# peternara/FashionVisualExpl-recommend

Measured on AMD Instinct MI355X. Metric: BPR triplets/sec, higher is better.
Workload: dtype bf16

## Files before the change

fashionvisualexpl_recommend_amd/_ffi.py:

```python
import ctypes as C
import os

HERE = os.path.dirname(os.path.abspath(__file__))
LIB_PATH = os.environ.get("BPRX_LIB") or os.path.join(HERE, "libbprx.so")
ABI_VERSION = 6
FLAG_EXPORT_USER_GRAD = 1
FLAG_EXPORT_ITEM_GRAD = 2
FLAG_DENSE_ALLREDUCE = 4
FLAG_ADAM_SWEEP, FLAG_ADAM_LAZY = 8, 16

MODEL = {"bprmf": 0, "vbpr": 1}
OPTIMIZER = {"sgd": 0, "adam_tf23": 1}
FEAT_DTYPE = {"fp32": 0, "bf16": 1, "fp8": 2}
E_INVALID, E_STATE = -1, -2
E_RANGE = -4
PHASES = ["cast_Et", "proj_fwd", "triplet_grad", "proj_bwd", "reduce_parts", "apply", "dense_update", "loss_reduce", "item_seg", "seg_alloc", "row_count", "adam_catchup"]


class BprxError(RuntimeError):
    def __init__(self, code, msg):
        super().__init__("libbprx error %d: %s" % (code, msg))
        self.code = code


class Config(C.Structure):
    _fields_ = [("abi_version", C.c_int32), ("model", C.c_int32), ("num_users", C.c_int32), ("num_items", C.c_int32),
                ("embed_k", C.c_int32), ("embed_d", C.c_int32), ("feat_dim", C.c_int32), ("feat_dtype", C.c_int32),
                ("optimizer", C.c_int32), ("device", C.c_int32), ("max_batch", C.c_int64),
                ("lr", C.c_float), ("reg", C.c_float), ("beta1", C.c_float), ("beta2", C.c_float),
                ("epsilon", C.c_float), ("flags", C.c_int32), ("feat_scale", C.c_float)]


FACTORED_FIELDS = ["Ea", "Eb", "A", "Ap", "m_Ea", "v_Ea", "m_Eb", "v_Eb", "m_A", "v_A", "m_Ap", "v_Ap"]


class Factored(C.Structure):
    _fields_ = [("feat_dim_a", C.c_int32), ("feat_dim_b", C.c_int32), ("embed_a", C.c_int32), ("embed_b", C.c_int32),
                ("neg_bias_reg", C.c_float)] + [(n, C.c_void_p) for n in FACTORED_FIELDS]


ACF_WEIGHTS = ["component.W_0_u", "component.W_0_i", "component.b_0", "component.W_1", "component.b_1",
               "item.W_0_u", "item.W_0_iv", "item.W_0_ip", "item.W_0_ix", "item.b_0", "item.W_1", "item.b_1"]


ACF_GRADIENT = {"detached": 0, "full": 1}


class Acf(C.Structure):
    _fields_ = [("feat_m", C.c_int32), ("feat_c", C.c_int32), ("width_c", C.c_int32), ("width_i", C.c_int32),
                ("feat_dtype", C.c_int32), ("F", C.c_void_p), ("train_ptr", C.c_void_p), ("train_items", C.c_void_p),
                ("eval_ptr", C.c_void_p), ("eval_items", C.c_void_p), ("Pi", C.c_void_p), ("m_Pi", C.c_void_p),
                ("v_Pi", C.c_void_p), ("w", C.c_void_p * 12), ("m_w", C.c_void_p * 12), ("v_w", C.c_void_p * 12)]


AF_WEIGHTS = ["color.W1", "color.b1", "color.W2", "edges.conv", "edges.conv_b", "edges.W2", "class.W1", "class.b1", "class.W2",
              "attention.W_1", "attention.b_1", "attention.W_2", "attention.b_2"]


class Attentive(C.Structure):
    _fields_ = [("dim_color", C.c_int32), ("dim_class", C.c_int32), ("width", C.c_int32), ("dropout", C.c_float),
                ("seed", C.c_uint64), ("edges", C.c_void_p), ("color", C.c_void_p), ("cls", C.c_void_p),
                ("w", C.c_void_p * 13), ("m_w", C.c_void_p * 13), ("v_w", C.c_void_p * 13)]


TABLE_FIELDS = ["Gu", "Gi", "Bi", "Tu", "F", "E", "Bp", "m_Gu", "v_Gu", "m_Gi", "v_Gi", "m_Bi", "v_Bi",
                "m_Tu", "v_Tu", "m_E", "v_E", "m_Bp", "v_Bp"]


class Tables(C.Structure):
    _fields_ = [(n, C.c_void_p) for n in TABLE_FIELDS]


_lib = None


def lib():
    global _lib
    if _lib is not None:
        return _lib
    import torch
    if not os.path.exists(LIB_PATH):
        raise ImportError("libbprx.so not found at %s: build it with `python -m fashionvisualexpl_recommend_amd.build` "
                          "(hipcc --offload-arch=gfx950); there is no CPU fallback" % LIB_PATH)
    L = C.CDLL(LIB_PATH)
    vp, i32, i64, u32, f32 = C.c_void_p, C.c_int32, C.c_int64, C.c_uint32, C.c_float
    sig = {
        "bprx_abi_version": (C.c_int, []),
        "bprx_create": (C.c_int, [C.POINTER(Config), C.POINTER(vp)]),
        "bprx_destroy": (C.c_int, [vp]),
        "bprx_last_error": (C.c_char_p, [vp]),
        "bprx_bind_tables": (C.c_int, [vp, C.POINTER(Tables)]),
        "bprx_bind_factored": (C.c_int, [vp, C.POINTER(Tables), C.POINTER(Factored)]),
        "bprx_explain_pairs": (C.c_int, [vp, vp, vp, i64, vp, vp]),
        "bprx_bind_acf": (C.c_int, [vp, C.POINTER(Tables), C.POINTER(Acf)]),
        "bprx_acf_profiles": (C.c_int, [vp, vp, i64, vp, vp, vp, vp]),
        "bprx_acf_explain": (C.c_int, [vp, vp, vp, i64, vp, vp, i32, vp, vp, vp, vp, vp, vp, vp, vp, vp, vp]),
        "bprx_acf_set_gradient": (C.c_int, [vp, C.c_int]),
        "bprx_acf_get_gradient": (C.c_int, [vp]),
        "bprx_bind_attentive": (C.c_int, [vp, C.POINTER(Tables), C.POINTER(Attentive)]),
        "bprx_af_encode": (C.c_int, [vp, vp, i64, vp, vp]),
        "bprx_af_attention_pairs": (C.c_int, [vp, vp, vp, i64, vp, vp, vp]),
        "bprx_af_explain": (C.c_int, [vp, vp, vp, i64, i32, vp, vp, vp, vp, vp, vp, vp]),
        "bprx_af_score_block": (C.c_int, [vp, C.c_int32, C.c_int32, vp, vp, vp]),
        "bprx_af_dropout_mask": (C.c_int, [vp, i64, i64, vp, vp]),
        "bprx_af_get_step": (i64, [vp]),
        "bprx_af_set_step": (C.c_int, [vp, i64]),
        "bprx_set_hyper": (C.c_int, [vp, f32, f32]),
        "bprx_tables_dirty": (C.c_int, [vp, vp]),
        "bprx_set_adam_step": (C.c_int, [vp, i64, vp]),
        "bprx_get_adam_step": (i64, [vp]),
        "bprx_adam_is_lazy": (C.c_int, [vp]),
        "bprx_sync_adam": (C.c_int, [vp, vp]),
        "bprx_score_pairs": (C.c_int, [vp, vp, vp, i64, vp, vp]),
        "bprx_step": (C.c_int, [vp, vp, vp, vp, i64, vp, vp]),
        "bprx_step_begin": (C.c_int, [vp, vp, vp, vp, i64, vp]),
        "bprx_step_begin_sparse": (C.c_int, [vp, vp, vp, vp, i64, vp]),
        "bprx_step_begin_dense": (C.c_int, [vp, vp]),
        "bprx_dense_grad": (C.c_int, [vp, C.POINTER(vp), C.POINTER(i64)]),
        "bprx_step_end": (C.c_int, [vp, vp, vp]),
        "bprx_step_project": (C.c_int, [vp, vp]),
        "bprx_user_grad": (C.c_int, [vp, C.POINTER(vp), C.POINTER(vp)]),
        "bprx_clear_user_grad": (C.c_int, [vp, i64, i32, vp]),
        "bprx_item_grad": (C.c_int, [vp, C.POINTER(vp), C.POINTER(vp)]),
        "bprx_clear_item_grad": (C.c_int, [vp, i64, i32, vp]),
        "bprx_scatter_add": (C.c_int, [vp, i32, i32, vp, vp, i64, f32, vp]),
        "bprx_route_reset": (C.c_int, [vp, i64, vp, i32, vp]),
        "bprx_route_plan": (C.c_int, [vp, i64, vp, i64, i32, i32, i32, i32, vp, vp, vp, vp, vp, vp]),
        "bprx_route_gather": (C.c_int, [vp, i32, vp, i32, i32, vp, i64, vp, vp, vp]),
        "bprx_route_unpack": (C.c_int, [vp, vp, i64, vp, i32, vp, i32, vp, vp, i32, vp]),
        "bprx_route_gather_checked": (C.c_int, [vp, i32, vp, i32, i32, vp, i64, vp, vp, vp, vp]),
        "bprx_route_unpack_checked": (C.c_int, [vp, vp, i64, vp, i32, vp, i32, vp, vp, i32, vp, vp]),
        "bprx_route_pack": (C.c_int, [vp, i32, vp, i32, vp, i64, vp, vp, vp, i32, f32, vp, vp, i64, vp, i32, vp]),
        "bprx_route_scatter_add": (C.c_int, [vp, i32, vp, i32, i32, vp, vp, i64, f32, vp, vp]),
        "bprx_score_block": (C.c_int, [vp, i32, i32, vp, vp]),
        "bprx_eval_users": (C.c_int, [vp, i32, i32, vp, vp, vp, vp, vp, i32, vp, vp]),
        "bprx_topk": (C.c_int, [vp, i32, i32, vp, vp, vp, i32, vp, vp, vp, vp]),
        "bprx_eval_pos": (C.c_int, [vp, i32, i32, vp, i32, i32, vp, vp, vp, vp]),
        "bprx_eval_counts": (C.c_int, [vp, i32, i32, vp, i32, i32, vp, vp, vp, vp, vp, vp, vp]),
        "bprx_eval_finish": (C.c_int, [vp, i32, i32, i32, vp, vp, vp, i32, vp, vp]),
        "bprx_sync_check": (C.c_int, [vp, vp]),
        "bprx_probe_stream_read": (i64, [vp, i64, vp, vp]),
        "bprx_probe_stream_read_nt": (i64, [vp, i64, vp, vp]),
        "bprx_probe_row_gather": (i64, [vp, i64, i32, vp, i64, i32, vp, vp]),
        "bprx_profile_enable": (C.c_int, [vp, C.c_int]),
        "bprx_profile_read": (C.c_int, [vp, vp, vp]),
        "bprx_sample_philox": (C.c_int, [vp, vp, vp, i64, i32, C.c_uint64, C.c_uint64, i64, vp, vp, vp, vp]),
        "bprx_user_msg_floats": (C.c_int64, [vp, i64]),
        "bprx_pack_user_msg": (C.c_int, [vp, vp, i64, i64, vp, vp]),
        "bprx_apply_user_msgs": (C.c_int, [vp, vp, i32, i64, C.c_float, vp]),
        "bprx_sum_dense_parts": (C.c_int, [vp, vp, i32, vp]),
        "bprx_epoch_prepare": (C.c_int, [C.c_uint64, u32, i32, vp, vp, vp, vp]),
        "bprx_epoch_slots": (C.c_int, [vp, i32, vp, i64, vp]),
        "bprx_sample_epoch": (C.c_int, [vp, vp, vp, vp, vp, i32, i32, C.c_uint64, u32, i64, i64, vp, vp, vp, vp]),
        "bprx_index_pass_kind": (C.c_int, [vp]),
        "bprx_adam_rows": (C.c_int, [vp, vp, vp, vp, i64, C.c_float, C.c_float, C.c_float, C.c_float, vp]),
        "bprx_step_lr": (C.c_int, [vp, vp]),
        "bprx_sample_philox_h": (C.c_int, [vp, vp, vp, vp, i64, i32, C.c_uint64, C.c_uint64, i64, vp, vp, vp, i64, i64, vp]),
        "bprx_sample_epoch_h": (C.c_int, [vp, vp, vp, vp, vp, vp, i32, i32, C.c_uint64, u32, i64, i64, vp, vp, vp, i64, i64, vp]),
        "bprx_sampler_create": (C.c_int, [vp, vp, i32, i32, C.POINTER(vp)]),
        "bprx_sampler_destroy": (C.c_int, [vp]),
        "bprx_sampler_count": (i64, [vp, i32, i32]),
        "bprx_sampler_ref_stream": (i64, [vp, i32, i32, u32, u32, vp, vp, vp, i64]),
    }
    for name, (res, args) in sig.items():
        fn = getattr(L, name)
        fn.restype, fn.argtypes = res, args
    if L.bprx_abi_version() != ABI_VERSION:
        raise ImportError("libbprx.so ABI %d != binding ABI %d" % (L.bprx_abi_version(), ABI_VERSION))
    _lib = L
    return L


EXPORTS = ["bprx_abi_version", "bprx_create", "bprx_destroy", "bprx_last_error", "bprx_bind_tables", "bprx_bind_factored", "bprx_explain_pairs", "bprx_bind_acf", "bprx_acf_profiles", "bprx_acf_explain", "bprx_acf_set_gradient", "bprx_acf_get_gradient", "bprx_bind_attentive", "bprx_af_encode", "bprx_af_attention_pairs", "bprx_af_explain",
           "bprx_af_score_block", "bprx_af_dropout_mask", "bprx_af_get_step", "bprx_af_set_step", "bprx_set_hyper", "bprx_tables_dirty",
           "bprx_set_adam_step", "bprx_get_adam_step", "bprx_adam_is_lazy", "bprx_sync_adam", "bprx_score_pairs", "bprx_step", "bprx_step_begin",
           "bprx_step_begin_sparse", "bprx_step_begin_dense", "bprx_sum_dense_parts",
           "bprx_dense_grad", "bprx_step_end", "bprx_step_project", "bprx_user_grad", "bprx_clear_user_grad", "bprx_item_grad", "bprx_clear_item_grad",
           "bprx_scatter_add", "bprx_route_reset", "bprx_route_plan", "bprx_route_gather", "bprx_route_unpack", "bprx_route_gather_checked",
           "bprx_route_unpack_checked", "bprx_route_pack",
           "bprx_route_scatter_add", "bprx_score_block", "bprx_eval_users", "bprx_eval_pos", "bprx_eval_counts", "bprx_eval_finish", "bprx_topk", "bprx_sync_check", "bprx_probe_stream_read", "bprx_probe_stream_read_nt", "bprx_probe_row_gather", "bprx_profile_enable",
           "bprx_profile_read", "bprx_sample_philox", "bprx_epoch_prepare", "bprx_epoch_slots", "bprx_sample_epoch", "bprx_sample_philox_h", "bprx_sample_epoch_h", "bprx_index_pass_kind", "bprx_adam_rows", "bprx_step_lr", "bprx_user_msg_floats", "bprx_pack_user_msg",
           "bprx_apply_user_msgs", "bprx_sampler_create",
           "bprx_sampler_destroy", "bprx_sampler_count", "bprx_sampler_ref_stream"]


def check(handle, rc):
    if rc < 0:
        msg = lib().bprx_last_error(handle)
        raise BprxError(rc, msg.decode() if msg else "?")
    return rc
```

fashionvisualexpl_recommend_amd/csrc/bprx_api.hip:

```cpp
#include <math.h>
#include <stdlib.h>
#include <algorithm>
#include <new>

#include "bprx_internal.h"
#include <utility>

static char g_create_err[512] = "";

static int check_ready(bprx_handle *h, int64_t B);

extern "C" int bprx_abi_version(void) { return BPRX_ABI_VERSION; }

extern "C" const char *bprx_last_error(const bprx_handle *h) { return h ? h->err : g_create_err; }

template <typename T>
static hipError_t dalloc_zero(T **p, size_t n) {
  *p = nullptr;
  if (n == 0) return hipSuccess;
  hipError_t e = hipMalloc((void **)p, n * sizeof(T));
  if (e != hipSuccess) return e;
  return hipMemset(*p, 0, n * sizeof(T));
}

static int env_int(const char *name, int fallback) {
  const char *e = getenv(name);
  return e ? atoi(e) : fallback;
}

static void free_scratch(bprx_handle *h) {
  void *ptrs[] = {h->dGu, h->dGi, h->dBi, h->dTu, h->flagU, h->flagI, h->lossb, h->loss_acc, h->errflag,
                  h->P,   h->W,   h->Wb, h->Ppair, h->Et, h->EtF, h->EtS, h->dEp, h->part, h->qs, h->Ft, h->seg_rank, h->seg_cnt, h->seg_ptr, h->seg_cursor, h->seg_lead, h->seg_ent, h->hot_done, h->uslot_of, h->ulist, h->uold, h->own8, h->loc8, h->cntU, h->cntI, h->ilist, h->ilist_n, h->lastU, h->lastI, h->lr_hist, h->slist, h->slist_n, h->msg_cursor, h->msg_next, h->gF};
  for (void *p : ptrs)
    if (p) (void)hipFree(p);
}

extern "C" int bprx_create(const bprx_config *cfg, bprx_handle **out) {
#define CFAIL(code, ...)                                        \
  do {                                                          \
    snprintf(g_create_err, sizeof(g_create_err), __VA_ARGS__);  \
    return (code);                                              \
  } while (0)
  if (!cfg || !out) CFAIL(BPRX_E_INVALID, "bprx_create: null argument");
  *out = nullptr;
  if (cfg->abi_version != BPRX_ABI_VERSION)
    CFAIL(BPRX_E_INVALID, "bprx_create: abi_version %d, library is %d", cfg->abi_version, BPRX_ABI_VERSION);
  if (cfg->model != BPRX_MODEL_BPRMF && cfg->model != BPRX_MODEL_VBPR) CFAIL(BPRX_E_INVALID, "unknown model %d", cfg->model);
  if (cfg->optimizer != BPRX_OPT_SGD && cfg->optimizer != BPRX_OPT_ADAM_TF23)
    CFAIL(BPRX_E_INVALID, "unknown optimizer %d", cfg->optimizer);
  if (cfg->num_users <= 0 || cfg->num_items <= 0 || cfg->embed_k <= 0 || cfg->max_batch <= 0)
    CFAIL(BPRX_E_INVALID, "num_users, num_items, embed_k and max_batch must be positive");
  const bool vb = cfg->model == BPRX_MODEL_VBPR;
  if (vb) {
    if (cfg->embed_d <= 0 || cfg->feat_dim <= 0) CFAIL(BPRX_E_INVALID, "VBPR needs embed_d > 0 and feat_dim > 0");
    if (cfg->embed_d > 271) CFAIL(BPRX_E_INVALID, "embed_d %d > 271 unsupported", cfg->embed_d);
    if (cfg->feat_dtype != BPRX_F_FP32 && cfg->feat_dtype != BPRX_F_BF16 && cfg->feat_dtype != BPRX_F_FP8)
      CFAIL(BPRX_E_INVALID, "unknown feat_dtype");
    if (cfg->feat_dtype == BPRX_F_BF16 && cfg->feat_dim % 128 != 0)
      CFAIL(BPRX_E_INVALID, "bf16 features need feat_dim %% 128 == 0 (got %d)", cfg->feat_dim);
    if (cfg->feat_dtype == BPRX_F_FP8 && cfg->feat_dim % 256 != 0)
      CFAIL(BPRX_E_INVALID, "fp8 features need feat_dim %% 256 == 0 (got %d)", cfg->feat_dim);
    if (cfg->feat_dtype == BPRX_F_FP8 && !(cfg->feat_scale > 0.f)) CFAIL(BPRX_E_INVALID, "fp8 features need feat_scale > 0");
  }
  const bool exported = cfg->flags & (BPRX_FLAG_EXPORT_USER_GRAD | BPRX_FLAG_EXPORT_ITEM_GRAD);
  bool adam_lazy = false;
  if (cfg->optimizer == BPRX_OPT_ADAM_TF23) {
    const double chain_us = 20.0 * (double)cfg->num_users / (double)cfg->max_batch * 0.45;
    const double sweep_us =
        ((double)cfg->num_users * (cfg->embed_k + (vb ? cfg->embed_d : 0)) + (double)cfg->num_items * (cfg->embed_k + 1)) * 24.0 / 4e6;
    adam_lazy = exported ? true : chain_us < sweep_us;
    if (cfg->flags & BPRX_FLAG_ADAM_SWEEP) adam_lazy = false;
    if (cfg->flags & BPRX_FLAG_ADAM_LAZY) adam_lazy = true;
    adam_lazy = env_int("BPRX_ADAM_LAZY", adam_lazy) != 0;
  }
  if (exported && cfg->optimizer != BPRX_OPT_SGD && !adam_lazy)
    CFAIL(BPRX_E_INVALID, "BPRX_FLAG_EXPORT_*_GRAD with adam_tf23 needs the lazy form (BPRX_ADAM_LAZY != 0)");
  if ((cfg->flags & BPRX_FLAG_EXPORT_ITEM_GRAD) && cfg->model != BPRX_MODEL_BPRMF)
    CFAIL(BPRX_E_INVALID, "BPRX_FLAG_EXPORT_ITEM_GRAD is for BPRMF (VBPR keeps its items and features local)");
  hipError_t e = hipSetDevice(cfg->device);
  if (e != hipSuccess) CFAIL(BPRX_E_HIP, "hipSetDevice(%d): %s", cfg->device, hipGetErrorString(e));

  bprx_handle *h = new (std::nothrow) bprx_handle();
  if (!h) CFAIL(BPRX_E_NOMEM, "out of host memory");
  memset(h, 0, sizeof(*h));
#define HFAIL(code, ...)         \
  do {                           \
    bprx_destroy(h);             \
    CFAIL(code, __VA_ARGS__);    \
  } while (0)
  h->cfg = *cfg;
  h->adam_lazy = adam_lazy;
  h->neg_bias_reg = 0.1f;
  if (!vb) { h->cfg.embed_d = 0; h->cfg.feat_dim = 0; }
  const size_t U = cfg->num_users, I = cfg->num_items, k = cfg->embed_k, d = h->cfg.embed_d, D = h->cfg.feat_dim;
  const size_t MB = cfg->max_batch;
  bool ok = true;
#define A(call) ok = ok && ((e = (call)) == hipSuccess)
  A(dalloc_zero(&h->dGu, U * k));
  A(dalloc_zero(&h->dGi, I * k));
  A(dalloc_zero(&h->dBi, I));
  A(dalloc_zero(&h->flagU, U));
  A(dalloc_zero(&h->flagI, I));
  A(dalloc_zero(&h->lossb, MB));
  A(dalloc_zero(&h->loss_acc, (size_t)BPRX_DENSE_BLOCKS));
  A(dalloc_zero(&h->errflag, (size_t)1));
  if (cfg->flags & BPRX_FLAG_EXPORT_USER_GRAD) A(dalloc_zero(&h->msg_cursor, (size_t)2));
  A(dalloc_zero(&h->cntU, U));
  A(dalloc_zero(&h->cntI, I));
  if (vb) {
    h->PS = 16 * (int)((d + 1 + 15) / 16);
    const size_t PS = h->PS;
    {
      hipDeviceProp_t prop;
      const int ncu = hipGetDeviceProperties(&prop, cfg->device) == hipSuccess ? prop.multiProcessorCount : 256;
      const int mr = (int)((D + 255) / 256);
      h->SK = (ncu + mr - 1) / mr;
      if (cfg->feat_dtype == BPRX_F_FP8 && PS / 16 <= 9) h->SK *= 2;
    }
    if (h->SK > 64) h->SK = 64;
    if (h->SK < 1) h->SK = 1;
    h->fwd_variant = env_int("BPRX_FWD_VARIANT", 4);
    A(dalloc_zero(&h->dTu, U * d));
    A(dalloc_zero(&h->P, I * PS));
    A(dalloc_zero(&h->W, I * PS));
    A(dalloc_zero((uint16_t **)&h->Wb, I * PS));
    A(dalloc_zero(&h->Ppair, MB * PS));
    A(dalloc_zero((uint16_t **)&h->Et, PS * D));
    A(dalloc_zero((uint16_t **)&h->EtF, PS * D));
    if (cfg->feat_dtype == BPRX_F_FP8 && PS / 16 >= 10) A(dalloc_zero((uint8_t **)&h->EtS, PS * D));
    A(dalloc_zero(&h->dEp, D * d + D));
    A(dalloc_zero(&h->part, (size_t)h->SK * D * PS));
    A(dalloc_zero(&h->qs, (size_t)4));
    if (cfg->feat_dtype != BPRX_F_FP32)
      A(dalloc_zero((uint8_t **)&h->Ft, (size_t)((I + 31) / 32 * 32) * D * (cfg->feat_dtype == BPRX_F_FP8 ? 1 : 2)));
  }
#undef A
  if (!ok) HFAIL(BPRX_E_NOMEM, "scratch allocation failed: %s", hipGetErrorString(e));
  {
    const bool fits = k % 4 == 0 && d % 4 == 0 && k <= 256 && d <= 256;
    h->seg_policy = (fits && !(cfg->flags & BPRX_FLAG_EXPORT_ITEM_GRAD)) ? std::min(std::max(env_int("BPRX_ITEM_MODE", 1), 0), 2) : 0;
    h->item_mode = 0;
    if (h->seg_policy) {
      h->seg_lead_cap = (int64_t)(I + 8192 + 4 * 1024 + 2 * MB / 64 + 64 + 64);
      h->seg_ent_cap = (int64_t)(6 * MB + 64 * 1024 + 2048);
      h->idx8_shift = 0;
      for (int sh = 8; sh <= 13 && !h->idx8_shift; ++sh)
        if ((((int64_t)I - 1) >> sh) <= 255) h->idx8_shift = sh;
      bool ok2 = dalloc_zero(&h->seg_rank, (size_t)2 * MB) == hipSuccess && dalloc_zero(&h->seg_cnt, I) == hipSuccess &&
                 dalloc_zero(&h->seg_ptr, I) == hipSuccess && dalloc_zero(&h->seg_cursor, (size_t)6) == hipSuccess &&
                 dalloc_zero((int4 **)&h->seg_lead, (size_t)h->seg_lead_cap) == hipSuccess &&
                 dalloc_zero(&h->hot_done, I) == hipSuccess && dalloc_zero((int2 **)&h->seg_ent, (size_t)h->seg_ent_cap) == hipSuccess &&
                 dalloc_zero(&h->uslot_of, U) == hipSuccess && dalloc_zero(&h->ulist, MB) == hipSuccess &&
                 dalloc_zero(&h->uold, MB * (k + d)) == hipSuccess &&
                 (!h->idx8_shift ||
                  (dalloc_zero(&h->own8, (size_t)2 * MB) == hipSuccess && dalloc_zero(&h->loc8, (size_t)2 * MB * (h->idx8_shift > 8 ? 2 : 1)) == hipSuccess));
      if (!ok2) HFAIL(BPRX_E_NOMEM, "segment scratch allocation failed");
    }
  }
  h->list_policy = vb ? std::min(std::max(env_int("BPRX_LIST_MODE", 1), 0), 2) : 0;
  if (h->list_policy) {
    const size_t cap = 2 * MB < I ? 2 * MB : I;
    if (dalloc_zero(&h->ilist, cap) != hipSuccess || dalloc_zero(&h->ilist_n, (size_t)2) != hipSuccess)
      HFAIL(BPRX_E_NOMEM, "item list allocation failed");
  }
  h->SK_step = h->SK;
  if (h->adam_lazy) {
    if (dalloc_zero(&h->lastU, U) != hipSuccess || dalloc_zero(&h->lastI, I) != hipSuccess ||
        dalloc_zero(&h->lr_hist, (size_t)bprx_adam_hist()) != hipSuccess)
      HFAIL(BPRX_E_NOMEM, "adam bookkeeping allocation failed");
  }
  h->fast_rows = (cfg->optimizer == BPRX_OPT_SGD && !(cfg->flags & BPRX_FLAG_EXPORT_USER_GRAD)) ? 1 : 0;
  if (h->fast_rows && !exported) {
    if (dalloc_zero(&h->slist, (size_t)3 * MB) != hipSuccess || dalloc_zero(&h->slist_n, (size_t)2) != hipSuccess)
      HFAIL(BPRX_E_NOMEM, "shared-row list allocation failed");
  }
  if (vb && cfg->optimizer == BPRX_OPT_ADAM_TF23 && h->adam_lazy && env_int("BPRX_SIDE_STREAM", 1) != 0 &&
      (hipStreamCreateWithFlags(&h->side, hipStreamNonBlocking) != hipSuccess ||
       hipEventCreateWithFlags(&h->ev_fork, hipEventDisableTiming) != hipSuccess ||
       hipEventCreateWithFlags(&h->ev_join, hipEventDisableTiming) != hipSuccess))
    HFAIL(BPRX_E_HIP, "side stream / event creation failed");
  {
    hipDeviceProp_t prop;
    h->num_cu = hipGetDeviceProperties(&prop, cfg->device) == hipSuccess ? prop.multiProcessorCount : 256;
  }
  h->prof_pending = new std::vector<bprx_handle::ProfRec>();
  h->prof_free = new std::vector<hipEvent_t>();
  *out = h;
  return BPRX_OK;
#undef HFAIL
#undef CFAIL
}

extern "C" int bprx_destroy(bprx_handle *h) {
  if (!h) return BPRX_OK;
  (void)hipSetDevice(h->cfg.device);
  if (h->side) (void)hipStreamSynchronize(h->side);
  free_scratch(h);
  bprx_acf_free(h);
  bprx_af_free(h);
  if (h->side) (void)hipStreamDestroy(h->side);
  if (h->ev_fork) (void)hipEventDestroy(h->ev_fork);
  if (h->ev_join) (void)hipEventDestroy(h->ev_join);
  if (h->prof_pending) { for (auto &r : *h->prof_pending) { (void)hipEventDestroy(r.a); (void)hipEventDestroy(r.b); } delete h->prof_pending; }
  if (h->prof_free) { for (auto e : *h->prof_free) (void)hipEventDestroy(e); delete h->prof_free; }
  delete h;
  return BPRX_OK;
}

extern "C" int bprx_profile_enable(bprx_handle *h, int on) {
  if (!h) return BPRX_E_INVALID;
  h->prof = on != 0;
  return BPRX_OK;
}

extern "C" int bprx_profile_read(bprx_handle *h, double *ms, int64_t *launches) {
  if (!h || !ms || !launches) return BPRX_E_INVALID;
  for (auto &r : *h->prof_pending) {
    BPRX_HIP(h, hipEventSynchronize(r.b));
    float t = 0.f;
    BPRX_HIP(h, hipEventElapsedTime(&t, r.a, r.b));
    ms[r.phase] += (double)t;
    launches[r.phase] += 1;
    h->prof_free->push_back(r.a);
    h->prof_free->push_back(r.b);
  }
  h->prof_pending->clear();
  return BPRX_OK;
}

static int bind_tables(bprx_handle *h, const bprx_tables *t, bool factored) {
  if (!h || !t) return BPRX_E_INVALID;
  if (!t->Gu || !t->Gi || !t->Bi) BPRX_FAIL(h, BPRX_E_INVALID, "bind_tables: Gu, Gi, Bi are required");
  const bool vb = h->cfg.model == BPRX_MODEL_VBPR;
  if (vb && (!t->Tu || !t->F || !t->E || !t->Bp)) BPRX_FAIL(h, BPRX_E_INVALID, "bind_tables: VBPR needs Tu, F, E, Bp");
  if (h->cfg.optimizer == BPRX_OPT_ADAM_TF23) {
    if (!t->m_Gu || !t->v_Gu || !t->m_Gi || !t->v_Gi || !t->m_Bi || !t->v_Bi)
      BPRX_FAIL(h, BPRX_E_INVALID, "bind_tables: adam_tf23 needs m_/v_ slots for Gu, Gi, Bi");
    if (vb && (!t->m_Tu || !t->v_Tu || (!factored && (!t->m_E || !t->v_E || !t->m_Bp || !t->v_Bp))))
      BPRX_FAIL(h, BPRX_E_INVALID, "bind_tables: adam_tf23 needs m_/v_ slots for Tu, E, Bp");
  }
  if (((uintptr_t)t->Gu | (uintptr_t)t->Gi | (uintptr_t)t->Tu | (uintptr_t)t->F | (uintptr_t)t->E) & 15)
    BPRX_FAIL(h, BPRX_E_INVALID, "bind_tables: table base pointers must be 16-byte aligned");
  h->t = *t;
  h->factored = factored;
  if (!factored) h->neg_bias_reg = 0.1f;
  h->et_valid = h->p_valid = h->absmax_valid = false;
  {
    const int rc = bprx_launch_tile_F(h);
    if (rc) return rc;
  }
  h->bound = true;
  return bprx_launch_adam_reset(h, h->adam_t, 0);
}

extern "C" int bprx_bind_tables(bprx_handle *h, const bprx_tables *t) {
  if (h && h->acf) bprx_acf_free(h);
  if (h && h->af) bprx_af_free(h);
  return bind_tables(h, t, false);
}

int bprx_bind_tables_internal(bprx_handle *h, const bprx_tables *t) { return bind_tables(h, t, false); }

extern "C" int bprx_bind_factored(bprx_handle *h, const bprx_tables *t, const bprx_factored *f) {
  if (!h || !t || !f) return BPRX_E_INVALID;
  const bprx_config &c = h->cfg;
  if (c.model != BPRX_MODEL_VBPR) BPRX_FAIL(h, BPRX_E_INVALID, "bind_factored: needs a VBPR handle");
  if (c.feat_dtype == BPRX_F_FP8) BPRX_FAIL(h, BPRX_E_INVALID, "bind_factored: fp8 features are not supported (fp32 or bf16)");
  if (c.flags & (BPRX_FLAG_EXPORT_USER_GRAD | BPRX_FLAG_EXPORT_ITEM_GRAD))
    BPRX_FAIL(h, BPRX_E_INVALID, "bind_factored: exported gradients (multi-GPU) are not supported");
  if (f->feat_dim_a <= 0 || f->feat_dim_b <= 0 || (int64_t)f->feat_dim_a + f->feat_dim_b > c.feat_dim)
    BPRX_FAIL(h, BPRX_E_INVALID, "bind_factored: need Dc, De > 0 and Dc + De <= feat_dim (%d, %d, %d)", f->feat_dim_a,
              f->feat_dim_b, c.feat_dim);
  if (f->embed_a <= 0 || f->embed_b <= 0 || f->embed_a > 256 || f->embed_b > 256)
    BPRX_FAIL(h, BPRX_E_INVALID, "bind_factored: embed_a, embed_b must lie in [1, 256] (%d, %d)", f->embed_a, f->embed_b);
  if (!(f->neg_bias_reg >= 0.f)) BPRX_FAIL(h, BPRX_E_INVALID, "bind_factored: neg_bias_reg must be >= 0");
  if (!f->Ea || !f->Eb || !f->A || !f->Ap) BPRX_FAIL(h, BPRX_E_INVALID, "bind_factored: Ea, Eb, A, Ap are required");
  if (c.optimizer == BPRX_OPT_ADAM_TF23 &&
      (!f->m_Ea || !f->v_Ea || !f->m_Eb || !f->v_Eb || !f->m_A || !f->v_A || !f->m_Ap || !f->v_Ap))
    BPRX_FAIL(h, BPRX_E_INVALID, "bind_factored: adam_tf23 needs m_/v_ slots for Ea, Eb, A, Ap");
  if (!h->gF) {
    const size_t n = (size_t)f->feat_dim_a * f->embed_a + (size_t)f->feat_dim_b * f->embed_b +
                     (size_t)(f->embed_a + f->embed_b) * (c.embed_d + 1);
    BPRX_HIP(h, hipMalloc((void **)&h->gF, n * sizeof(float)));
  } else if (f->feat_dim_a != h->fx.feat_dim_a || f->feat_dim_b != h->fx.feat_dim_b || f->embed_a != h->fx.embed_a ||
             f->embed_b != h->fx.embed_b) {
    BPRX_FAIL(h, BPRX_E_INVALID, "bind_factored: the factor shapes of a handle cannot change");
  }
  int rc = bind_tables(h, t, true);
  if (rc) return rc;
  h->fx = *f;
  h->neg_bias_reg = f->neg_bias_reg;
  if ((rc = bprx_launch_fact_compose(h, nullptr))) return rc;
  BPRX_HIP(h, hipStreamSynchronize(nullptr));
  return BPRX_OK;
}

extern "C" int bprx_explain_pairs(bprx_handle *h, const int32_t *user, const int32_t *item, int64_t n, float *out, void *stream) {
  int rc = check_ready(h, 0);
  if (rc) return rc;
  if (!h->factored) BPRX_FAIL(h, BPRX_E_STATE, "explain_pairs: the handle is not bound with bprx_bind_factored");
  if (n < 0 || n > ((int64_t)1 << 32)) BPRX_FAIL(h, BPRX_E_INVALID, "explain_pairs: n = %lld out of range", (long long)n);
  if (n == 0) return BPRX_OK;
  if (!user || !item || !out) BPRX_FAIL(h, BPRX_E_INVALID, "explain_pairs: null pointer");
  hipStream_t s = (hipStream_t)stream;
  if ((rc = bprx_launch_adam_sync(h, h->adam_t, s))) return rc;
  return bprx_launch_explain(h, user, item, n, out, s);
}

extern "C" int bprx_tables_dirty(bprx_handle *h, void *stream) {
  if (!h) return BPRX_E_INVALID;
  h->et_valid = h->p_valid = h->absmax_valid = false;
  if (h->acf) bprx_acf_invalidate(h);
  if (h->af) bprx_af_invalidate(h);
  if (h->bound && h->factored) {
    const int rc = bprx_launch_fact_compose(h, (hipStream_t)stream);
    if (rc) return rc;
  }
  return h->bound ? bprx_launch_adam_reset(h, h->adam_t, (hipStream_t)stream) : BPRX_OK;
}

extern "C" int bprx_set_hyper(bprx_handle *h, float lr, float reg) {
  if (!h) return BPRX_E_INVALID;
  h->cfg.lr = lr;
  h->cfg.reg = reg;
  return BPRX_OK;
}

extern "C" int bprx_set_adam_step(bprx_handle *h, int64_t it, void *stream) {
  if (!h || it < 0) return BPRX_E_INVALID;
  h->adam_t = it;
  return h->bound ? bprx_launch_adam_reset(h, it, (hipStream_t)stream) : BPRX_OK;
}

extern "C" int64_t bprx_get_adam_step(const bprx_handle *h) { return h ? h->adam_t : -1; }
extern "C" int bprx_adam_is_lazy(const bprx_handle *h) { return h ? (h->adam_lazy ? 1 : 0) : BPRX_E_INVALID; }

static int check_ready(bprx_handle *h, int64_t B) {
  if (!h) return BPRX_E_INVALID;
  if (!h->bound) BPRX_FAIL(h, BPRX_E_STATE, "tables not bound (call bprx_bind_tables first)");
  if (B < 0 || B > h->cfg.max_batch) BPRX_FAIL(h, BPRX_E_INVALID, "B=%lld outside [0, max_batch=%lld]", (long long)B, (long long)h->cfg.max_batch);
  return BPRX_OK;
}

extern "C" int bprx_sync_adam(bprx_handle *h, void *stream) {
  int rc = check_ready(h, 0);
  if (rc) return rc;
  return bprx_launch_adam_sync(h, h->adam_t, (hipStream_t)stream);
}

extern "C" int bprx_score_pairs(bprx_handle *h, const int32_t *user, const int32_t *item, int64_t B, float *x, void *stream) {
  int rc = check_ready(h, B);
  if (rc) return rc;
  if (B == 0) return BPRX_OK;
  if (!user || !item || !x) BPRX_FAIL(h, BPRX_E_INVALID, "score_pairs: null pointer");
  hipStream_t s = (hipStream_t)stream;
  if (h->acf) return bprx_acf_score_pairs(h, user, item, B, x, s);
  if (h->af) return bprx_af_pairs(h, user, item, B, x, nullptr, s);
  if ((rc = bprx_launch_adam_sync(h, h->adam_t, s))) return rc;
  if (h->cfg.model == BPRX_MODEL_VBPR) {
    if (h->p_valid) return bprx_launch_score(h, user, item, B, nullptr, 0, x, s);
    if ((rc = bprx_launch_cast_Et(h, s))) return rc;
    if ((rc = bprx_launch_proj_fwd(h, item, B, nullptr, 0, h->Ppair, s))) return rc;
    return bprx_launch_score(h, user, item, B, h->Ppair, 1, x, s);
  }
  return bprx_launch_score(h, user, item, B, nullptr, 0, x, s);
}

extern "C" int bprx_step_begin_sparse(bprx_handle *h, const int32_t *user, const int32_t *pos, const int32_t *neg, int64_t B, void *stream) {
  int rc = check_ready(h, B);
  if (rc) return rc;
  if (h->pending_stage) BPRX_FAIL(h, BPRX_E_STATE, "step_begin called twice without step_end");
  if (h->acf) BPRX_FAIL(h, BPRX_E_STATE, "step_begin: an ACF handle takes whole steps only (bprx_step)");
  if (h->af) BPRX_FAIL(h, BPRX_E_STATE, "step_begin: an AttentiveFashion handle takes whole steps only (bprx_step)");
  hipStream_t s = (hipStream_t)stream;
  const bool vb = h->cfg.model == BPRX_MODEL_VBPR;
  if (B == 0) {
    if (!(h->cfg.flags & (BPRX_FLAG_EXPORT_USER_GRAD | BPRX_FLAG_EXPORT_ITEM_GRAD))) BPRX_FAIL(h, BPRX_E_INVALID, "step: empty batch");
    h->list_mode = 0; h->item_mode = 0;
    if (h->cfg.optimizer == BPRX_OPT_ADAM_TF23) {
      h->adam_t += 1;
      const float t = (float)h->adam_t;
      const float lr_t = h->cfg.lr * sqrtf(1.0f - powf(h->cfg.beta2, t)) / (1.0f - powf(h->cfg.beta1, t));
      if (h->adam_lazy) {
        if (h->adam_t - h->adam_synced >= bprx_adam_hist() - 2 && (rc = bprx_launch_adam_sync(h, h->adam_t - 1, s))) return rc;
        if ((rc = bprx_launch_adam_catchup(h, nullptr, nullptr, nullptr, 0, lr_t, s))) return rc;
      }
      h->pend_lr = lr_t;
    } else h->pend_lr = h->cfg.lr;
    h->pending_B = 0; h->pending_stage = 1;
    h->pend_u = h->pend_i = h->pend_j = nullptr;
    return BPRX_OK;
  }
  if (!user || !pos || !neg) BPRX_FAIL(h, BPRX_E_INVALID, "step: null index pointer");
  h->list_mode = vb && !h->proj_fresh && (h->list_policy == 2 || (h->list_policy == 1 && 2 * B < (int64_t)h->cfg.num_items));
  h->item_mode = !h->list_mode && (h->seg_policy == 2 || (h->seg_policy == 1 && 2 * B >= (int64_t)h->cfg.num_items));
  h->list_reset_cnt = !(h->fast_rows && !(h->cfg.flags & BPRX_FLAG_EXPORT_ITEM_GRAD));
  h->idx8_use = h->idx8_ready(pos, neg, B);
  h->idx8_n = 0;
  float lr_t = h->cfg.lr;
  bool catchup_aside = false;
  if (h->cfg.optimizer == BPRX_OPT_ADAM_TF23) {
    h->adam_t += 1;
    float t = (float)h->adam_t;
    lr_t = h->cfg.lr * sqrtf(1.0f - powf(h->cfg.beta2, t)) / (1.0f - powf(h->cfg.beta1, t));
    if (h->adam_lazy) {
      if (h->adam_t - h->adam_synced >= bprx_adam_hist() - 2 && (rc = bprx_launch_adam_sync(h, h->adam_t - 1, s))) return rc;
      catchup_aside = h->side && !h->proj_fresh && !h->list_mode && !h->p_valid;
      if (!catchup_aside && (rc = bprx_launch_adam_catchup(h, user, pos, neg, B, lr_t, s))) return rc;
    }
  }
  if (catchup_aside) {
    BPRX_HIP(h, hipEventRecord(h->ev_fork, s));
    BPRX_HIP(h, hipStreamWaitEvent(h->side, h->ev_fork, 0));
    if ((rc = bprx_launch_adam_catchup(h, user, pos, neg, B, lr_t, h->side))) return rc;
    BPRX_HIP(h, hipEventRecord(h->ev_join, h->side));
  }
  if (h->list_mode) {
    h->list_cur = h->ilist_n + h->list_slot;
    h->list_bound = 2 * B < (int64_t)h->cfg.num_items ? 2 * B : (int64_t)h->cfg.num_items;
    if ((rc = bprx_launch_cast_Et(h, s))) return rc;
    if ((rc = bprx_launch_index_pass(h, user, pos, neg, B, s))) return rc;
    if (!h->p_valid &&
        (rc = bprx_launch_proj_fwd(h, h->ilist, h->list_bound, h->list_cur, 1, h->P, s))) return rc;
  } else if (vb && !h->proj_fresh) {
    if ((rc = bprx_launch_cast_Et(h, s))) return rc;
    if (!h->p_valid && (rc = bprx_launch_proj_fwd(h, nullptr, h->cfg.num_items, nullptr, 0, h->P, s))) return rc;
  }
  h->proj_fresh = false;
  if (catchup_aside) BPRX_HIP(h, hipStreamWaitEvent(s, h->ev_join, 0));
  if (!h->list_mode && (rc = bprx_launch_index_pass(h, user, pos, neg, B, s))) return rc;
  if ((rc = bprx_launch_triplet_grad(h, user, pos, neg, B, s))) return rc;
  h->pending_B = B;
  h->pending_stage = 1;
  h->pend_u = user; h->pend_i = pos; h->pend_j = neg; h->pend_lr = lr_t;
  return BPRX_OK;
}

extern "C" int bprx_step_begin_dense(bprx_handle *h, void *stream) {
  if (!h) return BPRX_E_INVALID;
  if (h->pending_stage != 1) BPRX_FAIL(h, BPRX_E_STATE, "step_begin_dense without step_begin_sparse");
  hipStream_t s = (hipStream_t)stream;
  const bool vb = h->cfg.model == BPRX_MODEL_VBPR;
  if (h->pending_B == 0) {
    if (vb) BPRX_HIP(h, hipMemsetAsync(h->dEp, 0, ((size_t)h->cfg.feat_dim * (h->cfg.embed_d + 1)) * sizeof(float), s));
    h->pending_stage = 2;
    return BPRX_OK;
  }
  const int32_t *user = h->pend_u, *pos = h->pend_i, *neg = h->pend_j;
  const int64_t B = h->pending_B;
  const float lr_t = h->pend_lr;
  int rc;
  if ((rc = bprx_launch_item_seg(h, pos, neg, B, lr_t, s))) return rc;
  if (vb && (rc = bprx_launch_proj_bwd(h, B, s))) return rc;
  if ((rc = bprx_launch_apply(h, user, pos, neg, B, lr_t, s))) return rc;
  h->pending_stage = 2;
  return BPRX_OK;
}

extern "C" int bprx_step_begin(bprx_handle *h, const int32_t *user, const int32_t *pos, const int32_t *neg, int64_t B, void *stream) {
  int rc = bprx_step_begin_sparse(h, user, pos, neg, B, stream);
  if (!rc && (rc = bprx_step_begin_dense(h, stream))) { h->pending_B = 0; h->pending_stage = 0; }
  return rc;
}

extern "C" int bprx_step_project(bprx_handle *h, void *stream) {
  int rc = check_ready(h, 0);
  if (rc) return rc;
  if (h->cfg.model != BPRX_MODEL_VBPR) return BPRX_OK;
  hipStream_t s = (hipStream_t)stream;
  if ((rc = bprx_launch_cast_Et(h, s))) return rc;
  if (!h->p_valid && (rc = bprx_launch_proj_fwd(h, nullptr, h->cfg.num_items, nullptr, 0, h->P, s))) return rc;
  h->p_valid = true;
  h->proj_fresh = true;
  return BPRX_OK;
}

extern "C" int bprx_user_grad(bprx_handle *h, float **dGu, float **dTu) {
  if (!h || !dGu || !dTu) return BPRX_E_INVALID;
  *dGu = h->dGu;
  *dTu = h->dTu;
  return BPRX_OK;
}

extern "C" int bprx_clear_user_grad(bprx_handle *h, int64_t n_rows, int32_t marks_only, void *stream) {
  if (!h || n_rows < 0 || n_rows > h->cfg.num_users) return BPRX_E_INVALID;
  hipStream_t s = (hipStream_t)stream;
  if (!marks_only) {
    BPRX_HIP(h, hipMemsetAsync(h->dGu, 0, (size_t)n_rows * h->cfg.embed_k * sizeof(float), s));
    if (h->cfg.embed_d) BPRX_HIP(h, hipMemsetAsync(h->dTu, 0, (size_t)n_rows * h->cfg.embed_d * sizeof(float), s));
  }
  BPRX_HIP(h, hipMemsetAsync(h->flagU, 0, (size_t)n_rows * sizeof(uint32_t), s));
  return BPRX_OK;
}

extern "C" int bprx_item_grad(bprx_handle *h, float **dGi, float **dBi) {
  if (!h || !dGi || !dBi) return BPRX_E_INVALID;
  *dGi = h->dGi;
  *dBi = h->dBi;
  return BPRX_OK;
}

extern "C" int bprx_clear_item_grad(bprx_handle *h, int64_t n_rows, int32_t marks_only, void *stream) {
  if (!h || n_rows < 0 || n_rows > h->cfg.num_items) return BPRX_E_INVALID;
  hipStream_t s = (hipStream_t)stream;
  if (!marks_only) {
    BPRX_HIP(h, hipMemsetAsync(h->dGi, 0, (size_t)n_rows * h->cfg.embed_k * sizeof(float), s));
    BPRX_HIP(h, hipMemsetAsync(h->dBi, 0, (size_t)n_rows * sizeof(float), s));
  }
  BPRX_HIP(h, hipMemsetAsync(h->flagI, 0, (size_t)n_rows * sizeof(uint32_t), s));
  return BPRX_OK;
}

extern "C" int bprx_dense_grad(bprx_handle *h, float **ptr, int64_t *count) {
  if (!h || !ptr || !count) return BPRX_E_INVALID;
  *ptr = h->dEp;
  *count = h->cfg.model == BPRX_MODEL_VBPR ? (int64_t)h->cfg.feat_dim * (h->cfg.embed_d + 1) : 0;
  return BPRX_OK;
}

extern "C" int bprx_step_end(bprx_handle *h, float *loss_out, void *stream) {
  if (!h) return BPRX_E_INVALID;
  if (!h->pending_stage) BPRX_FAIL(h, BPRX_E_STATE, "step_end without step_begin");
  if (h->pending_stage != 2) BPRX_FAIL(h, BPRX_E_STATE, "step_end before step_begin_dense");
  hipStream_t s = (hipStream_t)stream;
  int rc;
  float lr_t = h->cfg.lr;
  if (h->cfg.optimizer == BPRX_OPT_ADAM_TF23) {
    float t = (float)h->adam_t;
    lr_t = h->cfg.lr * sqrtf(1.0f - powf(h->cfg.beta2, t)) / (1.0f - powf(h->cfg.beta1, t));
  }
  int64_t B = h->pending_B;
  h->pending_B = 0;
  h->pending_stage = 0;
  if (h->factored && (rc = bprx_launch_fact_update(h, lr_t, s))) return rc;
  if (h->cfg.model == BPRX_MODEL_VBPR && (rc = bprx_launch_dense_update(h, lr_t, s))) return rc;
  if (loss_out && (rc = bprx_launch_loss_reduce(h, B, loss_out, s))) return rc;
  return BPRX_OK;
}

extern "C" int bprx_step(bprx_handle *h, const int32_t *user, const int32_t *pos, const int32_t *neg, int64_t B,
                         float *loss_out, void *stream) {
  if (!h) return BPRX_E_INVALID;
  if (h->acf) {
    const int rc = check_ready(h, B);
    return rc ? rc : bprx_acf_step(h, user, pos, neg, B, loss_out, (hipStream_t)stream);
  }
  if (h->af) {
    const int rc = check_ready(h, B);
    return rc ? rc : bprx_af_step(h, user, pos, neg, B, loss_out, (hipStream_t)stream);
  }
  h->fused_reduce = !h->factored;
  int rc = bprx_step_begin(h, user, pos, neg, B, stream);
  if (!rc) rc = bprx_step_end(h, loss_out, stream);
  h->fused_reduce = false;
  return rc;
}

extern "C" int bprx_score_block(bprx_handle *h, int32_t u0, int32_t u1, float *out, void *stream) {
  int rc = check_ready(h, 0);
  if (rc) return rc;
  if (u0 < 0 || u1 > h->cfg.num_users || u0 > u1 || !out) BPRX_FAIL(h, BPRX_E_INVALID, "score_block: bad user range [%d,%d)", u0, u1);
  if (u0 == u1) return BPRX_OK;
  hipStream_t s = (hipStream_t)stream;
  if ((rc = bprx_launch_adam_sync(h, h->adam_t, s))) return rc;
  if (h->af) return bprx_af_block(h, u0, u1, out, nullptr, s);
  if (h->acf) {
    if ((rc = bprx_acf_eval_profiles(h, s))) return rc;
    float *gu = h->t.Gu;
    h->t.Gu = bprx_acf_eval_gu(h);
    rc = h->cfg.embed_k % 2 == 0 ? bprx_launch_score_gemm(h, u0, u1, out, s) : bprx_launch_score_block(h, u0, u1, out, s);
    h->t.Gu = gu;
    return rc;
  }
  if (h->cfg.model == BPRX_MODEL_VBPR && !h->p_valid) {
    if ((rc = bprx_launch_cast_Et(h, s))) return rc;
    if ((rc = bprx_launch_proj_fwd(h, nullptr, h->cfg.num_items, nullptr, 0, h->P, s))) return rc;
    h->p_valid = true;
  }
  if (h->cfg.embed_k % 2 == 0 && h->cfg.embed_d % 2 == 0)
    return bprx_launch_score_gemm(h, u0, u1, out, s);
  return bprx_launch_score_block(h, u0, u1, out, s);
}

extern "C" int bprx_step_lr(const bprx_handle *h, float *lr_t) {
  if (!h || !lr_t) return BPRX_E_INVALID;
  *lr_t = h->pend_lr;
  return BPRX_OK;
}

extern "C" int bprx_index_pass_kind(const bprx_handle *h) { return h ? h->idx_kind : 0; }

extern "C" int bprx_sync_check(bprx_handle *h, void *stream) {
  if (!h) return BPRX_E_INVALID;
  hipStream_t s = (hipStream_t)stream;
  int32_t flag = 0;
  BPRX_HIP(h, hipMemcpyAsync(&flag, h->errflag, sizeof(flag), hipMemcpyDeviceToHost, s));
  BPRX_HIP(h, hipStreamSynchronize(s));
  if (flag) {
    BPRX_HIP(h, hipMemsetAsync(h->errflag, 0, sizeof(flag), s));
    BPRX_FAIL(h, BPRX_E_RANGE, "a user/item index was out of range (code %d); it was clamped, results are invalid", flag);
  }
  return BPRX_OK;
}
```

fashionvisualexpl_recommend_amd/csrc/bprx_internal.h:

```cpp
#pragma once
#include <hip/hip_runtime.h>
#include <stdint.h>
#include <stdio.h>
#include <string.h>

#include <vector>

#include "bprx.h"

#define BPRX_DENSE_BLOCKS 2048

struct AcfState;
struct AfState;

struct bprx_handle {
  bprx_config cfg;
  bprx_tables t;
  bool bound;
  int64_t adam_t;
  bool adam_lazy;
  int32_t *lastU, *lastI;
  float *lr_hist;
  int64_t adam_synced;
  char err[512];

  float *dGu, *dGi, *dBi, *dTu;
  uint32_t *flagU, *flagI;
  float *lossb;
  double *loss_acc;
  int dense_blocks;
  bool proj_fresh;
  bool et_valid;
  bool p_valid;
  bool fused_reduce;
  int32_t *errflag;
  int PS;
  float *P;
  float *W;
  void *Wb;
  float *Ppair;
  void *Ft;
  void *Et;
  void *EtF;
  void *EtS;
  float *dEp;
  float *part;
  int SK;
  float *qs;
  int qs_slot;
  bool absmax_valid;
  int fast_rows;
  int32_t *cntU, *cntI;
  int seg_policy;
  int item_mode;
  int32_t *seg_rank;
  int32_t *seg_cnt;
  int32_t *seg_ptr;
  int32_t *seg_cursor;
  int seg_slot;
  int seg_cur_slot;
  void *seg_lead;
  int64_t seg_lead_cap;
  int seg_lead_over;
  int64_t seg_ent_cap;
  int32_t *uslot_of;
  int32_t *ulist;
  float *uold;
  uint8_t *own8, *loc8;
  int idx8_shift;
  const int32_t *idx8_pos, *idx8_neg;
  int64_t idx8_B, idx8_n;
  bool idx8_use;
  int idx_kind;
  bool idx8_ready(const int32_t *pos, const int32_t *neg, int64_t B) const {
    return item_mode && own8 && B > 0 && idx8_n == B && idx8_B == B && idx8_pos == pos && idx8_neg == neg && B % 16 == 0;
  }
  int32_t *hot_done;
  void *seg_ent;
  int list_policy;
  int list_mode;
  int32_t *ilist;
  int32_t *ilist_n;
  int list_slot;
  int32_t *list_cur;
  int64_t list_bound;
  bool list_reset_cnt;
  bool W_dirty;
  int32_t *slist, *slist_n;
  int slist_slot;
  int SK_step;
  int num_cu;
  int fwd_variant;
  int64_t pending_B;
  int pending_stage;
  const int32_t *pend_u, *pend_i, *pend_j;
  float pend_lr;
  float neg_bias_reg;
  bool factored;
  bprx_factored fx;
  float *gF;
  struct AcfState *acf;
  struct AfState *af;
  int32_t *msg_cursor;
  int32_t *msg_next;
  size_t msg_next_n;
  hipStream_t side;
  hipEvent_t ev_fork, ev_join;
  bool prof;
  struct ProfRec { int phase; hipEvent_t a, b; };
  std::vector<ProfRec> *prof_pending;
  std::vector<hipEvent_t> *prof_free;
};

struct BprxProfScope {
  bprx_handle *h; hipStream_t s; hipEvent_t a, b; int phase; bool on;
  BprxProfScope(bprx_handle *h_, int phase_, hipStream_t s_) : h(h_), s(s_), phase(phase_), on(h_->prof) {
    if (!on) return;
    auto get = [&]() { hipEvent_t e; if (!h->prof_free->empty()) { e = h->prof_free->back(); h->prof_free->pop_back(); }
                       else (void)hipEventCreate(&e); return e; };
    a = get(); b = get();
    (void)hipEventRecord(a, s);
  }
  ~BprxProfScope() {
    if (!on) return;
    (void)hipEventRecord(b, s);
    h->prof_pending->push_back({phase, a, b});
  }
};

#define BPRX_FAIL(h, code, ...)                                   \
  do {                                                            \
    snprintf((h)->err, sizeof((h)->err), __VA_ARGS__);            \
    return (code);                                                \
  } while (0)

#define BPRX_HIP(h, call)                                                                          \
  do {                                                                                             \
    hipError_t e__ = (call);                                                                       \
    if (e__ != hipSuccess) BPRX_FAIL(h, BPRX_E_HIP, "%s: %s", #call, hipGetErrorString(e__));      \
  } while (0)

#define BPRX_LAUNCH_CHECK(h, name)                                                                 \
  do {                                                                                             \
    hipError_t e__ = hipGetLastError();                                                            \
    if (e__ != hipSuccess) BPRX_FAIL(h, BPRX_E_HIP, "launch %s: %s", name, hipGetErrorString(e__)); \
  } while (0)

int bprx_launch_score(bprx_handle *h, const int32_t *u, const int32_t *i, int64_t B, const float *Prow,
                      int p_by_pair, float *x, hipStream_t s);
int bprx_launch_index_pass(bprx_handle *h, const int32_t *u, const int32_t *i, const int32_t *j, int64_t B, hipStream_t s);
int bprx_launch_triplet_grad(bprx_handle *h, const int32_t *u, const int32_t *i, const int32_t *j, int64_t B,
                             hipStream_t s);
int bprx_launch_item_seg(bprx_handle *h, const int32_t *i, const int32_t *j, int64_t B, float lr_t, hipStream_t s);
int bprx_launch_apply(bprx_handle *h, const int32_t *u, const int32_t *i, const int32_t *j, int64_t B,
                      float lr_t, hipStream_t s);
int bprx_launch_dense_update(bprx_handle *h, float lr_t, hipStream_t s);
int bprx_launch_adam_catchup(bprx_handle *h, const int32_t *u, const int32_t *i, const int32_t *j, int64_t B, float lr_t,
                             hipStream_t s);
int bprx_launch_adam_sync(bprx_handle *h, int64_t t, hipStream_t s);
int bprx_launch_adam_reset(bprx_handle *h, int64_t t, hipStream_t s);
int bprx_adam_hist(void);
int bprx_launch_loss_reduce(bprx_handle *h, int64_t B, float *loss_out, hipStream_t s);
int bprx_launch_score_block(bprx_handle *h, int32_t u0, int32_t u1, float *out, hipStream_t s);
int bprx_launch_score_gemm(bprx_handle *h, int32_t u0, int32_t u1, float *out, hipStream_t s);
int bprx_launch_tile_F(bprx_handle *h);
int bprx_launch_cast_Et(bprx_handle *h, hipStream_t s);
int bprx_launch_proj_fwd(bprx_handle *h, const int32_t *rows, int64_t nrows, const int32_t *nrows_dev, int scatter, float *Pout,
                         hipStream_t s);
int bprx_launch_proj_bwd(bprx_handle *h, int64_t B, hipStream_t s);
int bprx_launch_fact_compose(bprx_handle *h, hipStream_t s);
int bprx_launch_fact_update(bprx_handle *h, float lr_t, hipStream_t s);
int bprx_launch_explain(bprx_handle *h, const int32_t *u, const int32_t *i, int64_t n, float *out, hipStream_t s);
int bprx_acf_step(bprx_handle *h, const int32_t *u, const int32_t *i, const int32_t *j, int64_t B, float *loss_out, hipStream_t s);
int bprx_acf_score_pairs(bprx_handle *h, const int32_t *u, const int32_t *i, int64_t B, float *x, hipStream_t s);
int bprx_acf_eval_profiles(bprx_handle *h, hipStream_t s);
float *bprx_acf_eval_gu(bprx_handle *h);
void bprx_acf_invalidate(bprx_handle *h);
void bprx_acf_free(bprx_handle *h);
int bprx_af_step(bprx_handle *h, const int32_t *u, const int32_t *i, const int32_t *j, int64_t B, float *loss_out, hipStream_t s);
int bprx_af_pairs(bprx_handle *h, const int32_t *u, const int32_t *i, int64_t n, float *x, float *alpha, hipStream_t s);
int bprx_af_block(bprx_handle *h, int32_t u0, int32_t u1, float *out, float *alpha, hipStream_t s);
void bprx_af_invalidate(bprx_handle *h);
void bprx_af_free(bprx_handle *h);

__device__ __forceinline__ void philox4x32_10(uint32_t c0, uint32_t c1, uint32_t c2, uint32_t c3, uint32_t k0, uint32_t k1,
                                              uint32_t (&out)[4]) {
#pragma unroll
  for (int r = 0; r < 10; ++r) {
    const uint32_t h0 = __umulhi(0xD2511F53u, c0), l0 = 0xD2511F53u * c0;
    const uint32_t h1 = __umulhi(0xCD9E8D57u, c2), l1 = 0xCD9E8D57u * c2;
    const uint32_t n0 = h1 ^ c1 ^ k0, n2 = h0 ^ c3 ^ k1;
    c0 = n0; c1 = l1; c2 = n2; c3 = l0;
    k0 += 0x9E3779B9u; k1 += 0xBB67AE85u;
  }
  out[0] = c0; out[1] = c1; out[2] = c2; out[3] = c3;
}

__device__ __forceinline__ void adam_elem(float &p, float &m, float &v, float g, float b1, float b2, float lr_t, float eps) {
#pragma clang fp contract(off)
  const float omb1 = 1.0f - b1, omb2 = 1.0f - b2;
  const float mt = m * b1 + g * omb1;
  const float vt = v * b2 + (g * g) * omb2;
  m = mt; v = vt;
  p = p - lr_t * mt / (sqrtf(vt) + eps);
}
```

fashionvisualexpl_recommend_amd/csrc/bprx_proj.hip:

```cpp
#include "bprx_internal.h"

namespace {

typedef __attribute__((ext_vector_type(8))) __bf16 bf16x8;
typedef __attribute__((ext_vector_type(4))) __bf16 bf16x4;
typedef __attribute__((ext_vector_type(4))) float f32x4;

__device__ __forceinline__ uint16_t f2bf(float x) {
  uint32_t u = __float_as_uint(x);
  u += 0x7fffu + ((u >> 16) & 1u);
  return (uint16_t)(u >> 16);
}

__device__ __forceinline__ uint32_t f2e4m3(float x) {
  const uint32_t u = __float_as_uint(x), sign = (u >> 24) & 0x80u, a = u & 0x7fffffffu;
  const float ax = __uint_as_float(a);
  if (ax < 0.015625f) return sign | (uint32_t)__builtin_rintf(ax * 512.0f);
  const uint32_t rr = a + 0x7ffffu + ((a >> 20) & 1u);
  const int e = (int)(rr >> 23) - 127;
  const uint32_t m = (rr >> 20) & 7u;
  if (e > 8 || (e == 8 && m == 7u)) return sign | 0x7eu;
  return sign | ((uint32_t)(e + 7) << 3) | m;
}

typedef __attribute__((ext_vector_type(4))) int i32x4_t;
typedef __attribute__((ext_vector_type(2))) long i64x2_t;
template <bool NT>
__device__ __forceinline__ i32x4_t ld_stream16(const void *p) {
  if constexpr (NT) return __builtin_nontemporal_load(reinterpret_cast<const i32x4_t *>(p));
  else return *reinterpret_cast<const i32x4_t *>(p);
}
template <bool F8>
__device__ __forceinline__ f32x4 mfma_frag(i32x4_t a, i32x4_t b, f32x4 c) {
  if constexpr (F8) {
    const i64x2_t av = __builtin_bit_cast(i64x2_t, a), bv = __builtin_bit_cast(i64x2_t, b);
    c = __builtin_amdgcn_mfma_f32_16x16x32_fp8_fp8(av.x, bv.x, c, 0, 0, 0);
    return __builtin_amdgcn_mfma_f32_16x16x32_fp8_fp8(av.y, bv.y, c, 0, 0, 0);
  } else {
    return __builtin_amdgcn_mfma_f32_16x16x32_bf16(__builtin_bit_cast(bf16x8, a), __builtin_bit_cast(bf16x8, b), c, 0, 0, 0);
  }
}

__global__ __launch_bounds__(256) void k_absmax(const float *__restrict__ E, size_t nE, const float *__restrict__ Bp, size_t nB,
                                                uint32_t *__restrict__ out) {
  uint32_t m = 0;
  for (size_t e = (size_t)blockIdx.x * 256 + threadIdx.x; e < nE + nB; e += (size_t)gridDim.x * 256) {
    const float v = e < nE ? E[e] : Bp[e - nE];
    const uint32_t a = __float_as_uint(v) & 0x7fffffffu;
    m = a > m ? a : m;
  }
#pragma unroll
  for (int o = 32; o > 0; o >>= 1) { const uint32_t v = __shfl_xor(m, o, 64); m = v > m ? v : m; }
  __shared__ uint32_t wm[4];
  if ((threadIdx.x & 63) == 0) wm[threadIdx.x >> 6] = m;
  __syncthreads();
  if (threadIdx.x == 0) {
    uint32_t b = wm[0];
    for (int w = 1; w < 4; ++w) b = wm[w] > b ? wm[w] : b;
    if (b) atomicMax(out, b);
  }
}

__global__ __launch_bounds__(256) void k_cast_Et8(const float *__restrict__ E, const float *__restrict__ Bp,
                                                  uint8_t *__restrict__ Et, uint8_t *__restrict__ EtF, uint8_t *__restrict__ EtS,
                                                  int D, int d, int PS, float *__restrict__ qs, float feat_scale, int slot) {
  __shared__ __attribute__((aligned(16))) uint8_t tile[288][16];
  const float amax = qs[2 + slot];
  const float sE = amax > 0.f ? 448.0f / amax : 1.0f;
  if (blockIdx.x == 0 && threadIdx.x == 0) { qs[1] = 1.0f / (feat_scale * sE); qs[2 + (slot ^ 1)] = 0.f; }
  const int k0 = blockIdx.x * 16, NT = PS >> 4;
  for (int idx = threadIdx.x; idx < 16 * PS; idx += 256) {
    const int kr = idx / PS, n = idx - kr * PS, kk = k0 + kr;
    float v = 0.f;
    if (kk < D) v = n < d ? E[(size_t)kk * d + n] : (n == d ? Bp[kk] : 0.f);
    tile[n][kr] = (uint8_t)f2e4m3(v * sE);
  }
  __syncthreads();
  for (int n = threadIdx.x; n < PS; n += 256) {
    const uint4 v = *reinterpret_cast<const uint4 *>(&tile[n][0]);
    const int b = k0 & 255, bs = k0 & 127;
    *reinterpret_cast<uint4 *>(Et + ((size_t)(k0 >> 8) * PS + n) * 256 + b) = v;
    *reinterpret_cast<uint4 *>(EtF + (((((size_t)(k0 >> 8) * 4 + (b >> 6)) * NT + (n >> 4)) * 64) + ((b >> 4) & 3) * 16 + (n & 15)) * 16) = v;
    if (EtS)
      *reinterpret_cast<uint4 *>(EtS + (((((size_t)(k0 >> 7) * NT + (n >> 4)) * 2 + ((bs >> 4) & 1)) * 64) + (bs >> 5) * 16 + (n & 15)) * 16) = v;
  }
}

__device__ __forceinline__ size_t et_idx(int n, int k, int PS) { return ((size_t)(k >> 7) * PS + n) * 128 + (k & 127); }

__device__ __forceinline__ size_t ft_row(int t, int Deq) { return ((size_t)(t >> 5) * (Deq >> 7)) * 4096 + (size_t)(t & 31) * 128; }
__device__ __forceinline__ size_t ft_col(int c) { return (size_t)(c >> 7) * 4096 + (c & 127); }

__global__ __launch_bounds__(256) void k_tile_F(const uint16_t *__restrict__ F, uint16_t *__restrict__ Ft, int I, int Deq) {
  const int cb = blockIdx.x, tb = blockIdx.y;
  uint4 *dst = reinterpret_cast<uint4 *>(Ft + ((size_t)tb * (Deq >> 7) + cb) * 4096);
  for (int p = threadIdx.x; p < 512; p += 256) {
    const int t = tb * 32 + (p >> 4);
    uint4 v = make_uint4(0, 0, 0, 0);
    if (t < I) v = *reinterpret_cast<const uint4 *>(F + (size_t)t * Deq + cb * 128 + (p & 15) * 8);
    dst[p] = v;
  }
}

__global__ __launch_bounds__(256) void k_cast_Et(const float *__restrict__ E, const float *__restrict__ Bp,
                                                 uint16_t *__restrict__ Et, uint16_t *__restrict__ EtF, int D, int d, int PS) {
  __shared__ float tile[64][17];
  const int k0 = blockIdx.x * 64, n0 = blockIdx.y * 16;
  for (int idx = threadIdx.x; idx < 64 * 16; idx += 256) {
    const int kr = idx >> 4, nc = idx & 15, kk = k0 + kr, n = n0 + nc;
    float v = 0.f;
    if (kk < D) v = n < d ? E[(size_t)kk * d + n] : (n == d ? Bp[kk] : 0.f);
    tile[kr][nc] = v;
  }
  __syncthreads();
  for (int idx = threadIdx.x; idx < 64 * 16; idx += 256) {
    const int nc = idx >> 6, kr = idx & 63, kk = k0 + kr, n = n0 + nc;
    if (n < PS && kk < D) {
      const uint16_t v = f2bf(tile[kr][nc]);
      Et[et_idx(n, kk, PS)] = v;
      const int e = kk & 127;
      EtF[(((((size_t)(kk >> 7) * 4 + (e >> 5)) * (PS >> 4) + (n >> 4)) * 64) + ((e >> 3) & 3) * 16 + (n & 15)) * 8 + (e & 7)] = v;
    }
  }
}

constexpr int KC = 128;
constexpr int BS_STRIDE = KC + 8;

template <int NT, int MT, bool F8>
__global__ __launch_bounds__(256) void k_proj_fwd_bf16(const uint16_t *__restrict__ F, const int32_t *__restrict__ rows,
                                                       int nrows, int nitems, int D, const uint16_t *__restrict__ Et,
                                                       float *__restrict__ P, int PS, int32_t *errflag, int stagger,
                                                       const float *__restrict__ pscale) {
  __shared__ __attribute__((aligned(16))) uint16_t Bs[NT * 16 * BS_STRIDE];
  const int lane = threadIdx.x & 63, w = threadIdx.x >> 6;
  const int r = lane & 15, q = lane >> 4;
  const int row0 = (blockIdx.x * 4 + w) * MT * 16;
  const int nchunks = D / KC;
  const int cshift = (stagger & 1) ? (int)((blockIdx.x >> 3) % (unsigned)nchunks) : 0;
  constexpr bool dbg_skip_b = false, dbg_skip_a = false;
  const uint16_t *arow[MT];
#pragma unroll
  for (int mt = 0; mt < MT; ++mt) {
    int t = row0 + mt * 16 + r;
    if (t >= nrows) t = nrows - 1;
    int item = rows ? rows[t] : t;
    if ((unsigned)item >= (unsigned)nitems) { *errflag = 2; item = 0; }
    arow[mt] = F + ft_row(item, D) + q * 8;
  }
  f32x4 acc[MT][NT];
#pragma unroll
  for (int mt = 0; mt < MT; ++mt)
#pragma unroll
    for (int nt = 0; nt < NT; ++nt) acc[mt][nt] = f32x4{0.f, 0.f, 0.f, 0.f};

  for (int cc = 0; cc < nchunks; ++cc) {
    int ce = cc + cshift;
    if (ce >= nchunks) ce -= nchunks;
    const int k0 = ce * KC;
    __syncthreads();
    if (!(dbg_skip_b && cc > 0))
    for (int idx = threadIdx.x; idx < NT * 16 * (KC / 8); idx += 256) {
      const int n = idx / (KC / 8), kk = (idx % (KC / 8)) * 8;
      *reinterpret_cast<uint4 *>(&Bs[n * BS_STRIDE + kk]) = *reinterpret_cast<const uint4 *>(&Et[et_idx(n, k0 + kk, NT * 16)]);
    }
    __syncthreads();
#pragma unroll
    for (int ks = 0; ks < KC; ks += 32) {
      bf16x8 a[MT];
#pragma unroll
      for (int mt = 0; mt < MT; ++mt) a[mt] = *reinterpret_cast<const bf16x8 *>(arow[mt] + ft_col(((dbg_skip_a && cc > 0) ? 0 : k0) + ks));
#pragma unroll
      for (int nt = 0; nt < NT; ++nt) {
        const bf16x8 b = *reinterpret_cast<const bf16x8 *>(&Bs[(nt * 16 + r) * BS_STRIDE + ks + q * 8]);
#pragma unroll
        for (int mt = 0; mt < MT; ++mt)
          acc[mt][nt] = mfma_frag<F8>(__builtin_bit_cast(i32x4_t, a[mt]), __builtin_bit_cast(i32x4_t, b), acc[mt][nt]);
      }
    }
  }
  const float ps = F8 ? *pscale : 1.0f;
#pragma unroll
  for (int mt = 0; mt < MT; ++mt)
#pragma unroll
    for (int reg = 0; reg < 4; ++reg) {
      const int t = row0 + mt * 16 + q * 4 + reg;
      if (t < nrows) {
#pragma unroll
        for (int nt = 0; nt < NT; ++nt) P[(size_t)t * PS + nt * 16 + r] = acc[mt][nt][reg] * ps;
      }
    }
}

template <int NTW, int MT, int NW, bool F8>
__global__ __launch_bounds__(NW * 64) void k_proj_fwd_rows(const uint16_t *__restrict__ F, const int32_t *__restrict__ rows,
                                                       int nrows, const int32_t *__restrict__ nrows_dev, int nitems, int D,
                                                       const uint16_t *__restrict__ EtF, float *__restrict__ P, int PS,
                                                       int32_t *errflag, const float *__restrict__ pscale, int scatter) {
  extern __shared__ __attribute__((aligned(16))) float red_rows[];
  constexpr int CG = NW == 16 ? 2 : (MT == 1 ? (NTW <= 9 ? 4 : (NTW <= 13 ? 2 : 1)) : (MT == 2 ? 2 : 1));
  constexpr int KS = KC / 32;
  if (nrows_dev) { const int n = *nrows_dev; nrows = n < nrows ? n : nrows; }
  const int row0 = blockIdx.x * (MT * 16);
  if (row0 >= nrows) return;
  const int NT = PS >> 4, nt0 = blockIdx.y * NTW;
  const int lane = threadIdx.x & 63, w = __builtin_amdgcn_readfirstlane(threadIdx.x >> 6);
  const int r = lane & 15, q = lane >> 4;
  const uint16_t *arow[MT];
#pragma unroll
  for (int mt = 0; mt < MT; ++mt) {
    int t = row0 + mt * 16 + r;
    if (t >= nrows) t = nrows - 1;
    int item = rows ? rows[t] : t;
    if ((unsigned)item >= (unsigned)nitems) { *errflag = 2; item = 0; }
    arow[mt] = F + ft_row(item, D) + q * 8;
  }
  f32x4 acc[MT][NTW];
#pragma unroll
  for (int mt = 0; mt < MT; ++mt)
#pragma unroll
    for (int nt = 0; nt < NTW; ++nt) acc[mt][nt] = f32x4{0.f, 0.f, 0.f, 0.f};
  const int nch = D / KC;
  const unsigned char *eb = reinterpret_cast<const unsigned char *>(EtF);
  uint32_t boff[NTW];
#pragma unroll
  for (int nt = 0; nt < NTW; ++nt) { const int n = nt0 + nt < NT ? nt0 + nt : NT - 1; boff[nt] = (uint32_t)(n * 64 + lane) * 16u; }
  const uint32_t kstep = (uint32_t)NT * 1024u;
  for (int c0 = w; c0 < nch; c0 += NW * CG) {
    i32x4_t a[CG][KS][MT];
#pragma unroll
    for (int cg = 0; cg < CG; ++cg) {
      int c = c0 + cg * NW;
      c = c < nch ? c : c0;
#pragma unroll
      for (int ks = 0; ks < KS; ++ks)
#pragma unroll
        for (int mt = 0; mt < MT; ++mt) a[cg][ks][mt] = *reinterpret_cast<const i32x4_t *>(arow[mt] + ((size_t)c << 12) + ks * 32);
    }
    i32x4_t b[2][NTW];
#pragma unroll
    for (int nt = 0; nt < NTW; ++nt) b[0][nt] = *reinterpret_cast<const i32x4_t *>(eb + ((uint32_t)(c0 * KS) * kstep + boff[nt]));
    __builtin_amdgcn_sched_barrier(0);
#pragma unroll
    for (int st = 0; st < CG * KS; ++st) {
      const int cg = st / KS, ks = st % KS;
      if (st + 1 < CG * KS) {
        const int cg1 = (st + 1) / KS, ks1 = (st + 1) % KS;
        int c1 = c0 + cg1 * NW;
        c1 = c1 < nch ? c1 : c0;
#pragma unroll
        for (int nt = 0; nt < NTW; ++nt)
          b[(st + 1) & 1][nt] = *reinterpret_cast<const i32x4_t *>(eb + ((uint32_t)(c1 * KS + ks1) * kstep + boff[nt]));
      }
      __builtin_amdgcn_sched_barrier(0);
      if (c0 + cg * NW < nch) {
#pragma unroll
        for (int nt = 0; nt < NTW; ++nt)
#pragma unroll
          for (int mt = 0; mt < MT; ++mt) acc[mt][nt] = mfma_frag<F8>(a[cg][ks][mt], b[st & 1][nt], acc[mt][nt]);
      }
      __builtin_amdgcn_sched_barrier(0);
    }
  }
  const float ps = F8 ? *pscale : 1.0f;
#pragma unroll
  for (int mt = 0; mt < MT; ++mt) {
#pragma unroll
    for (int half = NW / 2; half >= 1; half >>= 1) {
      if (w >= half && w < 2 * half) {
#pragma unroll
        for (int nt = 0; nt < NTW; ++nt)
#pragma unroll
          for (int reg = 0; reg < 4; ++reg) red_rows[(((w - half) * NTW + nt) * 4 + reg) * 64 + lane] = acc[mt][nt][reg];
      }
      __syncthreads();
      if (w < half) {
#pragma unroll
        for (int nt = 0; nt < NTW; ++nt)
#pragma unroll
          for (int reg = 0; reg < 4; ++reg) acc[mt][nt][reg] += red_rows[((w * NTW + nt) * 4 + reg) * 64 + lane];
      }
      __syncthreads();
    }
    if (w == 0) {
#pragma unroll
      for (int reg = 0; reg < 4; ++reg) {
        const int t = row0 + mt * 16 + q * 4 + reg;
        if (t < nrows) {
          int o = t;
          if (scatter) { o = rows[t]; if ((unsigned)o >= (unsigned)nitems) o = 0; }
#pragma unroll
          for (int nt = 0; nt < NTW; ++nt)
            if (nt0 + nt < NT) P[(size_t)o * PS + (nt0 + nt) * 16 + r] = acc[mt][nt][reg] * ps;
        }
      }
    }
  }
}

__device__ __forceinline__ bf16x4 lds_tr16(const uint16_t *p) {
  typedef __attribute__((ext_vector_type(4))) short s16x4;
  s16x4 v = __builtin_amdgcn_ds_read_tr16_b64_v4i16((__attribute__((address_space(3))) s16x4 *)p);
  return __builtin_bit_cast(bf16x4, v);
}

__global__ __launch_bounds__(256) void k_cast_W(float *__restrict__ W, uint16_t *__restrict__ Wb, size_t n4) {
  for (size_t e = (size_t)blockIdx.x * 256 + threadIdx.x; e < n4; e += (size_t)gridDim.x * 256) {
    float4 v = reinterpret_cast<float4 *>(W)[e];
    uint2 pk;
    pk.x = (uint32_t)f2bf(v.x) | ((uint32_t)f2bf(v.y) << 16);
    pk.y = (uint32_t)f2bf(v.z) | ((uint32_t)f2bf(v.w) << 16);
    reinterpret_cast<uint2 *>(Wb)[e] = pk;
    reinterpret_cast<float4 *>(W)[e] = make_float4(0.f, 0.f, 0.f, 0.f);
  }
}

template <int NT>
struct WsStride3 {
  static constexpr int bytes = ((NT * 32 + 128 - 32 + 255) / 256) * 256 + 32;
};

typedef __attribute__((ext_vector_type(2))) float f32x2_t;
typedef __attribute__((ext_vector_type(2))) __bf16 bf16x2_t;
__device__ __forceinline__ void fp8x4_to_bf16x4(uint32_t w, uint32_t &o0, uint32_t &o1) {
  o0 = __builtin_bit_cast(uint32_t, __builtin_amdgcn_cvt_scalef32_pk_bf16_fp8(w, 1.0f, false));
  o1 = __builtin_bit_cast(uint32_t, __builtin_amdgcn_cvt_scalef32_pk_bf16_fp8(w, 1.0f, true));
}

template <int NT, int BTV, int NW, int PD, bool F8, bool ROWS = false, int DB = 1, int NS = 1>
__global__ __launch_bounds__(NW * 64) void k_proj_bwd_bf16_v3(const uint16_t *__restrict__ F, int nrows, int D,
                                                          const uint16_t *__restrict__ Wb, int PS, float *__restrict__ part,
                                                          int rows_per_split, int descend, int xcd_map,
                                                          const int32_t *__restrict__ rows = nullptr,
                                                          const int32_t *__restrict__ nrows_dev = nullptr,
                                                          const float *__restrict__ Wf = nullptr) {
  constexpr int NTH = NW * 64, MC = NW * 32;
  constexpr int ESZ = F8 ? 1 : 2;
  constexpr int FCH = MC * ESZ / 16;
  constexpr int FSB = MC * 2 + 32;
  constexpr int WSB = WsStride3<NT>::bytes;
  constexpr int FPT = BTV * FCH / NTH;
  constexpr int CBK = MC * ESZ / 256;
  static_assert(CBK >= 1 && BTV % 32 == 0 && (BTV * FCH) % NTH == 0, "tile must be whole 8-KB blocks");
  constexpr int WCH = NT * 2;
  constexpr int WPT = (BTV * WCH + NTH - 1) / NTH;
  extern __shared__ __attribute__((aligned(16))) unsigned char lds_bwd3[];
  constexpr int IMG = BTV * FSB + BTV * WSB;
  unsigned char *const Fs0 = lds_bwd3, *const Ws0 = lds_bwd3 + BTV * FSB;
  const int lane = threadIdx.x & 63, w = threadIdx.x >> 6;
  const int g = lane >> 4, i16 = lane & 15, qq = i16 >> 2, p = i16 & 3;
  int bx = blockIdx.x, by = blockIdx.y;
  if (xcd_map && gridDim.y % 8 == 0) {
    const int flat = blockIdx.x + gridDim.x * blockIdx.y, xcd = flat & 7, slot = flat >> 3;
    by = (slot / (int)gridDim.x) * 8 + xcd;
    bx = slot % (int)gridDim.x;
  }
  const int m0 = bx * MC;
  const int Deq = D * ESZ / 2, m0q = m0 * ESZ / 2;
  if constexpr (ROWS) {
    const int n = *nrows_dev;
    nrows = n < nrows ? n : nrows;
    rows_per_split = ((nrows + (int)gridDim.y - 1) / (int)gridDim.y + BTV - 1) / BTV * BTV;
  }
  const int tbeg = by * rows_per_split;
  int tend = tbeg + rows_per_split;
  if (tend > nrows) tend = nrows;
  const int ntiles = tend > tbeg ? (tend - tbeg + BTV - 1) / BTV : 0;
  static_assert(NW % NS == 0, "wave grid");
  constexpr int MTW = 2 * NS, NTW = (NT + NS - 1) / NS;
  const int wm = w / NS, wn = w % NS;
  f32x4 acc[MTW][NTW];
#pragma unroll
  for (int mt = 0; mt < MTW; ++mt)
#pragma unroll
    for (int nt = 0; nt < NTW; ++nt) acc[mt][nt] = f32x4{0.f, 0.f, 0.f, 0.f};
  uint4 freg[PD][FPT], wreg[PD][WPT];
  uint4 wreg2[ROWS ? PD : 1][WPT];
#define BWD3_ISSUE(ST, TILE)                                                                                             \
  {                                                                                                                      \
    int tile_ = (TILE);                                                                                                  \
    tile_ = tile_ < ntiles ? tile_ : ntiles - 1;                                                                         \
    const int t0 = tbeg + (descend ? (ntiles - 1 - tile_) : tile_) * BTV;                                                \
     \
    _Pragma("unroll") for (int x = 0; x < FPT; ++x) {                                                                    \
      const int pp = threadIdx.x + x * NTH, blk = pp >> 9;                                                               \
      if constexpr (ROWS) {                                                                                              \
        int tp = t0 + (blk / CBK) * 32 + ((pp & 511) >> 4);                                                              \
        tp = tp < tend ? tp : tend - 1;                                                                                  \
        const int item = rows[tp];                                                                                       \
        freg[ST][x] = *reinterpret_cast<const uint4 *>(F + ft_row(item, Deq) + (size_t)((m0q >> 7) + blk % CBK) * 4096 + \
                                                       (size_t)(pp & 15) * 8);                                           \
      } else {                                                                                                           \
        const size_t bidx = (size_t)((t0 >> 5) + blk / CBK) * (Deq >> 7) + (m0q >> 7) + blk % CBK;                       \
        { const i32x4_t v_ = ld_stream16<!F8>(F + bidx * 4096 + (size_t)(pp & 511) * 8);                                 \
          freg[ST][x] = make_uint4((unsigned)v_.x, (unsigned)v_.y, (unsigned)v_.z, (unsigned)v_.w); }                      \
      }                                                                                                                  \
    }                                                                                                                    \
    _Pragma("unroll") for (int x = 0; x < WPT; ++x) {                                                                    \
      int idx = threadIdx.x + x * NTH;                                                                                   \
      idx = idx < BTV * WCH ? idx : BTV * WCH - 1;                                                                       \
      const int tr = idx / WCH, ch = idx % WCH;                                                                          \
      int t = t0 + tr;                                                                                                   \
      t = t < tend ? t : tend - 1;                                                                                       \
      if constexpr (ROWS) {                                                                                              \
        const float *wr = Wf + (size_t)rows[t] * PS + ch * 8;                                                            \
        wreg[ST][x] = *reinterpret_cast<const uint4 *>(wr);                                                              \
        wreg2[ST][x] = *reinterpret_cast<const uint4 *>(wr + 4);                                                         \
      } else {                                                                                                           \
        wreg[ST][x] = *reinterpret_cast<const uint4 *>(Wb + (size_t)t * PS + ch * 8);                                    \
      }                                                                                                                  \
    }                                                                                                                    \
  }
#define BWD3_COMMIT(ST, TILE)                                                                                            \
  {                                                                                                                      \
    const int tile_ = (TILE);                                                                                            \
    unsigned char *const Fs = Fs0 + (DB == 2 ? (tile_ & 1) * IMG : 0), *const Ws = Ws0 + (DB == 2 ? (tile_ & 1) * IMG : 0); \
    const int t0 = tile_ < ntiles ? tbeg + (descend ? (ntiles - 1 - tile_) : tile_) * BTV : tend;                        \
    const bool part_ = t0 + BTV > tend;                 \
    _Pragma("unroll") for (int x = 0; x < FPT; ++x) {                                                                    \
      const int pp = threadIdx.x + x * NTH, blk = pp >> 9;                                                               \
      const int tr = (blk / CBK) * 32 + ((pp & 511) >> 4), ch = (blk % CBK) * 16 + (pp & 15);                            \
      uint4 v = freg[ST][x];                                                                                             \
      if (part_) {                                                                                                       \
        const uint32_t mk = (t0 + tr < tend) ? 0xffffffffu : 0u;                                                         \
        v.x &= mk; v.y &= mk; v.z &= mk; v.w &= mk;                                                                      \
      }                                                                                                                  \
      if constexpr (F8) {                                                                                                \
        uint4 lo, hi;                                                                                                    \
        fp8x4_to_bf16x4(v.x, lo.x, lo.y); fp8x4_to_bf16x4(v.y, lo.z, lo.w);                                              \
        fp8x4_to_bf16x4(v.z, hi.x, hi.y); fp8x4_to_bf16x4(v.w, hi.z, hi.w);                                              \
        *reinterpret_cast<uint4 *>(&Fs[tr * FSB + ((ch * 32) ^ ((tr & 8) << 4))]) = lo;                                  \
        *reinterpret_cast<uint4 *>(&Fs[tr * FSB + ((ch * 32 + 16) ^ ((tr & 8) << 4))]) = hi;                             \
      } else {                                                                                                           \
        *reinterpret_cast<uint4 *>(&Fs[tr * FSB + ((ch * 16) ^ ((tr & 8) << 4))]) = v;                                   \
      }                                                                                                                  \
    }                                                                                                                    \
    _Pragma("unroll") for (int x = 0; x < WPT; ++x) {                                                                    \
      const int idx = threadIdx.x + x * NTH, tr = idx / WCH, ch = idx % WCH;                                             \
      uint4 v = wreg[ST][x];                                                                                             \
      if constexpr (ROWS) {                                                                                              \
        const uint4 u = wreg2[ST][x];                                                                                    \
        v.x = (uint32_t)f2bf(__uint_as_float(v.x)) | ((uint32_t)f2bf(__uint_as_float(v.y)) << 16);                       \
        v.y = (uint32_t)f2bf(__uint_as_float(v.z)) | ((uint32_t)f2bf(__uint_as_float(v.w)) << 16);                       \
        v.z = (uint32_t)f2bf(__uint_as_float(u.x)) | ((uint32_t)f2bf(__uint_as_float(u.y)) << 16);                       \
        v.w = (uint32_t)f2bf(__uint_as_float(u.z)) | ((uint32_t)f2bf(__uint_as_float(u.w)) << 16);                       \
      }                                                                                                                  \
      if (part_) {                                                                                                       \
        const uint32_t mk = (t0 + tr < tend) ? 0xffffffffu : 0u;                                                         \
        v.x &= mk; v.y &= mk; v.z &= mk; v.w &= mk;                                                                      \
      }                                                                                                                  \
      if (idx < BTV * WCH) *reinterpret_cast<uint4 *>(&Ws[tr * WSB + ((tr & 8) << 4) + ch * 16]) = v;                    \
    }                                                                                                                    \
  }
  if (ntiles == 0) {
    float *slab0 = part + ((size_t)by * D + m0) * PS;
    for (int e = threadIdx.x; e < MC * PS; e += NTH) slab0[e] = 0.f;
    return;
  }
#pragma unroll
  for (int st = 0; st < PD; ++st) BWD3_ISSUE(st, st)
  for (int tile0 = 0; tile0 < ntiles; tile0 += PD) {
#pragma unroll
   for (int st = 0; st < PD; ++st) {
    if (DB == 1) __syncthreads();
    BWD3_COMMIT(st, tile0 + st)
    __syncthreads();
    BWD3_ISSUE(st, tile0 + st + PD)
    const unsigned char *const Fs = Fs0 + (DB == 2 ? ((tile0 + st) & 1) * IMG : 0), *const Ws = Ws0 + (DB == 2 ? ((tile0 + st) & 1) * IMG : 0);
#pragma unroll
    for (int kk = 0; kk < BTV / 32; ++kk) {
      const int rlo = kk * 32 + 8 * g + qq, rhi = rlo + 4;
      const int disp = (g & 1) << 7;
      bf16x8 a[MTW];
#pragma unroll
      for (int mt = 0; mt < MTW; ++mt) {
        const int cb = (((wm * MTW + mt) * 16 + 4 * p) * 2) ^ disp;
        bf16x4 lo = lds_tr16(reinterpret_cast<const uint16_t *>(&Fs[rlo * FSB + cb]));
        bf16x4 hi = lds_tr16(reinterpret_cast<const uint16_t *>(&Fs[rhi * FSB + cb]));
        a[mt] = __builtin_shufflevector(lo, hi, 0, 1, 2, 3, 4, 5, 6, 7);
      }
#pragma unroll
      for (int nt = 0; nt < NTW; ++nt) {
        if (NS > 1 && wn * NTW + nt >= NT) break;
        const int cb = ((wn * NTW + nt) * 16 + 4 * p) * 2 + disp;
        bf16x4 lo = lds_tr16(reinterpret_cast<const uint16_t *>(&Ws[rlo * WSB + cb]));
        bf16x4 hi = lds_tr16(reinterpret_cast<const uint16_t *>(&Ws[rhi * WSB + cb]));
        const bf16x8 b = __builtin_shufflevector(lo, hi, 0, 1, 2, 3, 4, 5, 6, 7);
#pragma unroll
        for (int mt = 0; mt < MTW; ++mt) acc[mt][nt] = __builtin_amdgcn_mfma_f32_16x16x32_bf16(a[mt], b, acc[mt][nt], 0, 0, 0);
      }
    }
   }
  }
#undef BWD3_ISSUE
#undef BWD3_COMMIT
  float *slab = part + ((size_t)by * D + m0) * PS;
#pragma unroll
  for (int mt = 0; mt < MTW; ++mt)
#pragma unroll
    for (int reg = 0; reg < 4; ++reg) {
      const int m = (wm * MTW + mt) * 16 + g * 4 + reg;
#pragma unroll
      for (int nt = 0; nt < NTW; ++nt)
        if (NS == 1 || wn * NTW + nt < NT) slab[(size_t)m * PS + (wn * NTW + nt) * 16 + i16] = acc[mt][nt][reg];
    }
}


template <int NT, int MT, bool F8, bool NTL>
__device__ __forceinline__ void v10_body(const uint16_t *const (&asrc)[2], const uint16_t *__restrict__ Et, unsigned char *lds,
                                         unsigned char *myA, f32x4 (&acc)[2][NT], int D, int cshift, int lane, int et_chunk) {
  constexpr int BSB = (KC + 16) * 2;
  constexpr int BBUF = NT * 16 * BSB;
  constexpr int KS = KC / 32;
  constexpr int NPIECE = NT * 16 * (KC / 8);
  const int tid = threadIdx.x, bdim = (int)blockDim.x;
  const int r = lane & 15, q = lane >> 4;
  const int nch = D / KC;
  i32x4_t aX[MT][4], aY[MT][4];
  constexpr int NBR = (NPIECE + 319) / 320;
  i32x4_t bst[NBR];
#define V10_ISSUE(c_, AR)                                                                                             \
  {                                                                                                                   \
    int ce_ = (c_) + cshift;                                                                                          \
    if (ce_ >= nch) ce_ -= nch;                                                                                       \
    _Pragma("unroll") for (int mt = 0; mt < MT; ++mt) _Pragma("unroll") for (int x = 0; x < 4; ++x)                   \
        AR[mt][x] = ld_stream16<NTL>(asrc[mt] + ((size_t)ce_ << 12) + x * 512 + lane * 8);                          \
    const uint16_t *bc_ = Et + (size_t)ce_ * et_chunk;                                                                \
    _Pragma("unroll") for (int x = 0; x < NBR; ++x) {                                                                 \
      int pc = tid + x * bdim;                                                                                        \
      pc = pc < NPIECE ? pc : NPIECE - 1;                                                                             \
      bst[x] = *reinterpret_cast<const i32x4_t *>(bc_ + pc * 8);                                                      \
    }                                                                                                                 \
  }
#define V10_PARK(buf_)                                                                                                \
  {                                                                                                                   \
    _Pragma("unroll") for (int x = 0; x < NBR; ++x) {                                                                 \
      int pc = tid + x * bdim;                                                                                        \
      pc = pc < NPIECE ? pc : NPIECE - 1;                                                                             \
      *reinterpret_cast<i32x4_t *>(lds + (buf_) * BBUF + (pc / (KC / 8)) * BSB + (pc % (KC / 8)) * 16) = bst[x];      \
    }                                                                                                                 \
  }
#define V10_COMPUTE(buf_, AR)                                                                                         \
  {                                                                                                                   \
             \
    _Pragma("unroll") for (int mt = 0; mt < MT; ++mt) _Pragma("unroll") for (int x = 0; x < 4; ++x)                   \
        *reinterpret_cast<i32x4_t *>(myA + (mt * 16 + x * 4 + (lane >> 4)) * BSB + (lane & 15) * 16) = AR[mt][x];      \
    i32x4_t af[KS][MT];                                                                                               \
    _Pragma("unroll") for (int ks = 0; ks < KS; ++ks) _Pragma("unroll") for (int mt = 0; mt < MT; ++mt)               \
        af[ks][mt] = *reinterpret_cast<const i32x4_t *>(myA + (mt * 16 + r) * BSB + ks * 64 + q * 16);                \
    const unsigned char *bl_ = lds + (buf_) * BBUF + r * BSB + q * 16;                                                \
    _Pragma("unroll") for (int ks = 0; ks < KS; ++ks) {                                                               \
      _Pragma("unroll") for (int nt = 0; nt < NT; ++nt) {                                                             \
        const i32x4_t b = *reinterpret_cast<const i32x4_t *>(bl_ + nt * 16 * BSB + ks * 64);                          \
        _Pragma("unroll") for (int mt = 0; mt < MT; ++mt) acc[mt][nt] = mfma_frag<F8>(af[ks][mt], b, acc[mt][nt]);    \
      }                                                                                                               \
    }                                                                                                                 \
  }
  V10_ISSUE(0, aX)
  V10_PARK(0)
  __syncthreads();
  for (int c = 0; c < nch; c += 2) {
    V10_ISSUE(c + 1, aY)
    __builtin_amdgcn_sched_barrier(0);
    V10_COMPUTE(0, aX)
    __builtin_amdgcn_sched_barrier(0);
    V10_PARK(1)
    __syncthreads();
    const int cn = c + 2 < nch ? c + 2 : nch - 1;
    V10_ISSUE(cn, aX)
    __builtin_amdgcn_sched_barrier(0);
    V10_COMPUTE(1, aY)
    __builtin_amdgcn_sched_barrier(0);
    V10_PARK(0)
    __syncthreads();
  }
#undef V10_ISSUE
#undef V10_PARK
#undef V10_COMPUTE
}

template <int NT, bool F8, bool NTL>
__global__ __launch_bounds__(512) void k_proj_fwd_bf16_v10(const uint16_t *__restrict__ F, int nrows, int D,
                                                           const uint16_t *__restrict__ Et, float *__restrict__ P, int PS,
                                                           const float *__restrict__ pscale, int stagger, int tiles_per_wave,
                                                           int n0) {
  extern __shared__ __attribute__((aligned(16))) unsigned char lds_v10[];
  constexpr int BSB = (KC + 16) * 2;
  const int lane = threadIdx.x & 63, w = __builtin_amdgcn_readfirstlane(threadIdx.x >> 6);
  const int r = lane & 15, q = lane >> 4;
  const int T = (nrows + 15) >> 4;
  const int t0 = (int)(((long long)blockIdx.x * T) / gridDim.x), t1 = (int)(((long long)(blockIdx.x + 1) * T) / gridDim.x);
  const int first = t0 + w * tiles_per_wave;
  const int nlive = (first < t1 ? 1 : 0) + ((tiles_per_wave == 2 && first + 1 < t1) ? 1 : 0);
  const uint16_t *asrc[2];
#pragma unroll
  for (int mt = 0; mt < 2; ++mt) {
    int tile = first + mt;
    if (tile >= t1) tile = t1 > t0 ? t1 - 1 : 0;
    asrc[mt] = F + ft_row(tile * 16, D);
  }
  f32x4 acc[2][NT];
#pragma unroll
  for (int mt = 0; mt < 2; ++mt)
#pragma unroll
    for (int nt = 0; nt < NT; ++nt) acc[mt][nt] = f32x4{0.f, 0.f, 0.f, 0.f};
  const int nch = D / KC;
  const int cshift = (stagger & 1) ? (int)(blockIdx.x % (unsigned)nch) : 0;
  unsigned char *myA = lds_v10 + 2 * NT * 16 * BSB + w * (2 * 16 * BSB);
  if (nlive == 2) v10_body<NT, 2, F8, NTL>(asrc, Et + (size_t)n0 * 128, lds_v10, myA, acc, D, cshift, lane, PS * 128);
  else v10_body<NT, 1, F8, NTL>(asrc, Et + (size_t)n0 * 128, lds_v10, myA, acc, D, cshift, lane, PS * 128);
  const float ps = F8 ? *pscale : 1.0f;
#pragma unroll
  for (int mt = 0; mt < 2; ++mt) {
    if (mt >= nlive) continue;
#pragma unroll
    for (int reg = 0; reg < 4; ++reg) {
      const int t = (first + mt) * 16 + q * 4 + reg;
      if (t < nrows) {
#pragma unroll
        for (int nt = 0; nt < NT; ++nt) P[(size_t)t * PS + n0 + nt * 16 + r] = acc[mt][nt][reg] * ps;
      }
    }
  }
}

typedef __attribute__((ext_vector_type(8))) int i32x8_t;

template <int NT, int MT, bool NTL>
__device__ __forceinline__ void f8s_body(const unsigned char *const (&arow)[2][2], const unsigned char *__restrict__ EtS,
                                         unsigned char *lds, unsigned char *myA, int nch, int cshift, int lane,
                                         float *__restrict__ P, int PS, int nrows, int first, int nstore, float ps,
                                         const int32_t *__restrict__ rows, int scatter, int nitems) {
  constexpr int BCH = NT * 2048;
  constexpr int NPIECE = NT * 128;
  constexpr int NBP = (NPIECE + 511) / 512;
  const int tid = threadIdx.x;
  f32x4 acc[MT][NT];
#pragma unroll
  for (int mt = 0; mt < MT; ++mt)
#pragma unroll
    for (int nt = 0; nt < NT; ++nt) acc[mt][nt] = f32x4{0.f, 0.f, 0.f, 0.f};
  i32x8_t aX[MT], aY[MT];
  i32x4_t bst[NBP];
  const int i_w = lane >> 3, p_w = lane & 7, i_r = lane & 15, g_r = lane >> 4;
  const int wo0 = i_w * 128 + ((p_w ^ (i_w & 7)) << 4);
  const int wo1 = (8 + i_w) * 128 + ((p_w ^ (i_w & 7) ^ 1) << 4);
  const int sw_r = (i_r & 7) ^ (i_r >> 3);
  const int ro0 = i_r * 128 + (((2 * g_r) ^ sw_r) << 4), ro1 = i_r * 128 + (((2 * g_r + 1) ^ sw_r) << 4);
#define F8S_ISSUE(c_, AR)                                                                                             \
  {                                                                                                                   \
    int ce_ = (c_) + cshift;                                                                                          \
    if (ce_ >= nch) ce_ -= nch;                                                                                       \
    const size_t ao_ = (size_t)(ce_ >> 1) * 8192 + (size_t)(ce_ & 1) * 128;                                           \
    _Pragma("unroll") for (int mt = 0; mt < MT; ++mt) {                                                               \
      AR[mt].lo = ld_stream16<NTL>(arow[mt][0] + ao_);                                                                \
      AR[mt].hi = ld_stream16<NTL>(arow[mt][1] + ao_);                                                                \
    }                                                                                                                 \
    const unsigned char *bc_ = EtS + (size_t)ce_ * BCH;                                                               \
    _Pragma("unroll") for (int x = 0; x < NBP; ++x) {                                                                 \
      int pc = tid + x * 512;                                                                                         \
      pc = pc < NPIECE ? pc : NPIECE - 1;                                                                             \
      bst[x] = *reinterpret_cast<const i32x4_t *>(bc_ + pc * 16);                                                     \
    }                                                                                                                 \
  }
#define F8S_PARK(buf_)                                                                                                \
  {                                                                                                                   \
    _Pragma("unroll") for (int x = 0; x < NBP; ++x) {                                                                 \
      int pc = tid + x * 512;                                                                                         \
      pc = pc < NPIECE ? pc : NPIECE - 1;                                                                             \
      *reinterpret_cast<i32x4_t *>(lds + (buf_) * BCH + pc * 16) = bst[x];                                            \
    }                                                                                                                 \
  }
#define F8S_COMPUTE(buf_, AR)                                                                                         \
  {                                                                                                                   \
                          \
    _Pragma("unroll") for (int mt = 0; mt < MT; ++mt) {                                                               \
      *reinterpret_cast<i32x4_t *>(myA + mt * 2048 + wo0) = AR[mt].lo;                                                \
      *reinterpret_cast<i32x4_t *>(myA + mt * 2048 + wo1) = AR[mt].hi;                                                \
    }                                                                                                                 \
    _Pragma("unroll") for (int mt = 0; mt < MT; ++mt) {                                                               \
      AR[mt].lo = *reinterpret_cast<const i32x4_t *>(myA + mt * 2048 + ro0);                                          \
      AR[mt].hi = *reinterpret_cast<const i32x4_t *>(myA + mt * 2048 + ro1);                                          \
    }                                                                                                                 \
                                                          \
    const unsigned char *bl_ = lds + (buf_) * BCH + lane * 16;                                                        \
    i32x8_t bq[2];                                                                                                    \
    bq[0].lo = *reinterpret_cast<const i32x4_t *>(bl_);                                                               \
    bq[0].hi = *reinterpret_cast<const i32x4_t *>(bl_ + 1024);                                                        \
    _Pragma("unroll") for (int nt = 0; nt < NT; ++nt) {                                                               \
      if (nt + 1 < NT) {                                                                                              \
        bq[(nt + 1) & 1].lo = *reinterpret_cast<const i32x4_t *>(bl_ + (nt + 1) * 2048);                              \
        bq[(nt + 1) & 1].hi = *reinterpret_cast<const i32x4_t *>(bl_ + (nt + 1) * 2048 + 1024);                       \
      }                                                                                                               \
      __builtin_amdgcn_sched_barrier(0);                                                                              \
      _Pragma("unroll") for (int mt = 0; mt < MT; ++mt)                                                               \
        acc[mt][nt] = __builtin_amdgcn_mfma_scale_f32_16x16x128_f8f6f4(AR[mt], bq[nt & 1], acc[mt][nt], 0, 0, 0,      \
                                                                       0x7f7f7f7f, 0, 0x7f7f7f7f);                    \
      __builtin_amdgcn_sched_barrier(0);                                                                              \
    }                                                                                                                 \
  }
  F8S_ISSUE(0, aX)
  F8S_PARK(0)
  __syncthreads();
  for (int c = 0; c < nch; c += 2) {
    F8S_ISSUE(c + 1, aY)
    __builtin_amdgcn_sched_barrier(0);
    F8S_COMPUTE(0, aX)
    F8S_PARK(1)
    __syncthreads();
    const int cn = c + 2 < nch ? c + 2 : nch - 1;
    F8S_ISSUE(cn, aX)
    __builtin_amdgcn_sched_barrier(0);
    F8S_COMPUTE(1, aY)
    F8S_PARK(0)
    __syncthreads();
  }
#undef F8S_ISSUE
#undef F8S_PARK
#undef F8S_COMPUTE
  const int r = lane & 15, g = lane >> 4;
#pragma unroll
  for (int mt = 0; mt < MT; ++mt) {
    if (mt >= nstore) continue;
#pragma unroll
    for (int reg = 0; reg < 4; ++reg) {
      const int t = (first + mt) * 16 + g * 4 + reg;
      if (t < nrows) {
        int orow = t;
        if (scatter) { orow = rows[t]; orow = (unsigned)orow < (unsigned)nitems ? orow : 0; }
#pragma unroll
        for (int nt = 0; nt < NT; ++nt) P[(size_t)orow * PS + nt * 16 + r] = acc[mt][nt][reg] * ps;
      }
    }
  }
}

template <int NT, bool NTL>
__global__ __launch_bounds__(512) void k_proj_fwd_f8s(const unsigned char *__restrict__ F, int nrows, int D,
                                                      const unsigned char *__restrict__ EtS, float *__restrict__ P, int PS,
                                                      const float *__restrict__ pscale, int stagger,
                                                      const int32_t *__restrict__ rows, const int32_t *__restrict__ nrows_dev,
                                                      int scatter, int nitems, int32_t *__restrict__ errflag) {
  extern __shared__ __attribute__((aligned(16))) unsigned char lds_f8s[];
  const int lane = threadIdx.x & 63, w = __builtin_amdgcn_readfirstlane(threadIdx.x >> 6);
  if (nrows_dev) { const int n = *nrows_dev; nrows = n < nrows ? n : nrows; }
  if (nrows <= 0) return;
  const int T = (nrows + 15) >> 4;
  const int t0 = (int)(((long long)blockIdx.x * T) / gridDim.x), t1 = (int)(((long long)(blockIdx.x + 1) * T) / gridDim.x);
  const int ntile = t1 - t0;
  if (ntile == 0) return;
  const int base = ntile >> 3, rem = ntile & 7;
  const int nlive = base + (w < rem ? 1 : 0);
  const int first = t0 + w * base + (w < rem ? w : rem);
  const unsigned char *arow[2][2];
#pragma unroll
  for (int mt = 0; mt < 2; ++mt) {
    int tile = first + mt;
    if (mt >= nlive) tile = nlive ? first + nlive - 1 : (T ? T - 1 : 0);
#pragma unroll
    for (int x = 0; x < 2; ++x) {
      int t = tile * 16 + 8 * x + (lane >> 3);
      if (t >= nrows) t = nrows - 1;
      if (rows) {
        t = rows[t];
        if ((unsigned)t >= (unsigned)nitems) { *errflag = 2; t = 0; }
      }
      arow[mt][x] = F + ((size_t)(t >> 5) * (size_t)(D >> 8)) * 8192 + (size_t)(t & 31) * 256 + (lane & 7) * 16;
    }
  }
  const int nch = D >> 7;
  const int cshift = (stagger & 1) ? (int)(blockIdx.x % (unsigned)nch) : 0;
  const float ps = *pscale;
  unsigned char *myA = lds_f8s + 2 * NT * 2048 + w * 4096;
  if (nlive == 2) f8s_body<NT, 2, NTL>(arow, EtS, lds_f8s, myA, nch, cshift, lane, P, PS, nrows, first, 2, ps, rows, scatter, nitems);
  else f8s_body<NT, 1, NTL>(arow, EtS, lds_f8s, myA, nch, cshift, lane, P, PS, nrows, first, nlive, ps, rows, scatter, nitems);
}

__global__ __launch_bounds__(256) void k_reduce_parts(const float *__restrict__ part, int SK, int D, int d, int PS,
                                                      float *__restrict__ dEp, float gscale) {
  const size_t e = (size_t)blockIdx.x * 256 + threadIdx.x;
  if (e >= (size_t)D * PS) return;
  const int kk = (int)(e / PS), n = (int)(e % PS);
  if (n > d) return;
  float s = 0.f;
  for (int sidx = 0; sidx < SK; ++sidx) s += part[(size_t)sidx * D * PS + e];
  s *= gscale;
  if (n < d) dEp[(size_t)kk * d + n] = s;
  else dEp[(size_t)D * d + kk] = s;
}

__global__ __launch_bounds__(256) void k_proj_fwd_f32(const float *__restrict__ F, const int32_t *__restrict__ rows,
                                                      int nrows, const int32_t *__restrict__ nrows_dev, int scatter, int nitems,
                                                      int D, const float *__restrict__ E, const float *__restrict__ Bp, int d,
                                                      float *__restrict__ P, int PS, int32_t *errflag) {
  const int t = blockIdx.x * 4 + (threadIdx.x >> 6), lane = threadIdx.x & 63;
  if (nrows_dev) { const int n = *nrows_dev; nrows = n < nrows ? n : nrows; }
  if (t >= nrows) return;
  int item = rows ? rows[t] : t;
  if ((unsigned)item >= (unsigned)nitems) { *errflag = 2; item = 0; }
  const float *f = F + (size_t)item * D;
  const size_t o = scatter ? (size_t)item : (size_t)t;
  for (int n = lane; n <= d; n += 64) {
    double acc = 0.0;
    if (n < d) for (int kk = 0; kk < D; ++kk) acc += (double)f[kk] * (double)E[(size_t)kk * d + n];
    else for (int kk = 0; kk < D; ++kk) acc += (double)f[kk] * (double)Bp[kk];
    P[o * PS + n] = (float)acc;
  }
}

__global__ __launch_bounds__(256) void k_proj_bwd_f32(const float *__restrict__ F, int nrows, int D,
                                                      const float *__restrict__ W, int d, int PS, float *__restrict__ dEp,
                                                      const int32_t *__restrict__ rows, const int32_t *__restrict__ nrows_dev) {
  const int kk = blockIdx.x;
  if (nrows_dev) { const int n = *nrows_dev; nrows = n < nrows ? n : nrows; }
  for (int n = threadIdx.x; n <= d; n += 256) {
    double acc = 0.0;
    if (rows) {
      for (int t = 0; t < nrows; ++t) {
        const int item = rows[t];
        acc += (double)F[(size_t)item * D + kk] * (double)W[(size_t)item * PS + n];
      }
    } else {
      for (int t = 0; t < nrows; ++t) acc += (double)F[(size_t)t * D + kk] * (double)W[(size_t)t * PS + n];
    }
    if (n < d) dEp[(size_t)kk * d + n] = (float)acc;
    else dEp[(size_t)D * d + kk] = (float)acc;
  }
}

constexpr int F32_NRS = 32, F32_KV = 8;
__global__ __launch_bounds__(1024) void k_proj_bwd_f32_tile(const float *__restrict__ F, int nrows, int D,
                                                            const float *__restrict__ W, int d, int PS, float *__restrict__ dEp,
                                                            const int32_t *__restrict__ rows, const int32_t *__restrict__ nrows_dev) {
  __shared__ double red[F32_NRS][F32_KV][32];
  if (nrows_dev) { const int n = *nrows_dev; nrows = n < nrows ? n : nrows; }
  const int rs = threadIdx.x >> 5, n = threadIdx.x & 31, col = blockIdx.y * 32 + n, k0 = blockIdx.x * F32_KV;
  double acc[F32_KV];
#pragma unroll
  for (int q = 0; q < F32_KV; ++q) acc[q] = 0.0;
  const bool on = col <= d;
  constexpr int RPT = 4;
  for (int t = rs; t < nrows; t += RPT * F32_NRS) {
    int item[RPT];
    double w[RPT];
    float4 v[RPT][2];
#pragma unroll
    for (int x = 0; x < RPT; ++x) {
      const int tx = t + x * F32_NRS;
      item[x] = rows ? rows[tx < nrows ? tx : t] : (tx < nrows ? tx : t);
    }
#pragma unroll
    for (int x = 0; x < RPT; ++x) {
      const float wv = on ? W[(size_t)item[x] * PS + col] : 0.f;
      w[x] = t + x * F32_NRS < nrows ? (double)wv : 0.0;
      const float *fr = F + (size_t)item[x] * D + k0;
      v[x][0] = *reinterpret_cast<const float4 *>(fr); v[x][1] = *reinterpret_cast<const float4 *>(fr + 4);
    }
#pragma unroll
    for (int x = 0; x < RPT; ++x) {
      acc[0] += (double)v[x][0].x * w[x]; acc[1] += (double)v[x][0].y * w[x]; acc[2] += (double)v[x][0].z * w[x]; acc[3] += (double)v[x][0].w * w[x];
      acc[4] += (double)v[x][1].x * w[x]; acc[5] += (double)v[x][1].y * w[x]; acc[6] += (double)v[x][1].z * w[x]; acc[7] += (double)v[x][1].w * w[x];
    }
  }
#pragma unroll
  for (int q = 0; q < F32_KV; ++q) red[rs][q][n] = acc[q];
  __syncthreads();
  if (on && rs < F32_KV) {
    const int q = rs;
    double sum = red[0][q][n];
    for (int x = 1; x < F32_NRS; ++x) sum += red[x][q][n];
    const int kk = k0 + q;
    if (col < d) dEp[(size_t)kk * d + col] = (float)sum;
    else dEp[(size_t)D * d + kk] = (float)sum;
  }
}

typedef double f64x4_t __attribute__((ext_vector_type(4)));
__global__ __launch_bounds__(1024) void k_proj_fwd_f32_mfma(const float *__restrict__ F, const int32_t *__restrict__ rows,
                                                            int nrows, const int32_t *__restrict__ nrows_dev, int scatter,
                                                            int nitems, int D, const float *__restrict__ E,
                                                            const float *__restrict__ Bp, int d, float *__restrict__ P, int PS,
                                                            int32_t *errflag) {
  __shared__ double red[16][4][64];
  if (nrows_dev) { const int n = *nrows_dev; nrows = n < nrows ? n : nrows; }
  const int t0 = blockIdx.x * 16;
  if (t0 >= nrows) return;
  const int w = threadIdx.x >> 6, lane = threadIdx.x & 63, i = lane & 15, kq = lane >> 4;
  const int t = t0 + i < nrows ? t0 + i : nrows - 1;
  int item = rows ? rows[t] : t;
  if ((unsigned)item >= (unsigned)nitems) { *errflag = 2; item = 0; }
  const float *fa = F + (size_t)item * D + 4 * kq;
  const int col = blockIdx.y * 16 + i;
  const bool isE = col < d, isB = col == d;
  f64x4_t acc = {0.0, 0.0, 0.0, 0.0};
  const int nchunk = D >> 4;
  constexpr int PT = 4;
  for (int c = w; c < nchunk; c += 16 * PT) {
    int kbx[PT];
    double wx[PT];
    float4 ax[PT];
    float bx[PT][4];
#pragma unroll
    for (int x = 0; x < PT; ++x) {
      const bool in = c + 16 * x < nchunk;
      kbx[x] = (in ? c + 16 * x : c) << 4;
      wx[x] = in ? 1.0 : 0.0;
    }
#pragma unroll
    for (int x = 0; x < PT; ++x) {
      ax[x] = *reinterpret_cast<const float4 *>(fa + kbx[x]);
#pragma unroll
      for (int s4 = 0; s4 < 4; ++s4) {
        const int kk = kbx[x] + 4 * kq + s4;
        bx[x][s4] = isE ? E[(size_t)kk * d + col] : (isB ? Bp[kk] : 0.f);
      }
    }
#pragma unroll
    for (int x = 0; x < PT; ++x) {
      acc = __builtin_amdgcn_mfma_f64_16x16x4f64((double)ax[x].x * wx[x], (double)bx[x][0], acc, 0, 0, 0);
      acc = __builtin_amdgcn_mfma_f64_16x16x4f64((double)ax[x].y * wx[x], (double)bx[x][1], acc, 0, 0, 0);
      acc = __builtin_amdgcn_mfma_f64_16x16x4f64((double)ax[x].z * wx[x], (double)bx[x][2], acc, 0, 0, 0);
      acc = __builtin_amdgcn_mfma_f64_16x16x4f64((double)ax[x].w * wx[x], (double)bx[x][3], acc, 0, 0, 0);
    }
  }
  red[w][0][lane] = acc.x; red[w][1][lane] = acc.y; red[w][2][lane] = acc.z; red[w][3][lane] = acc.w;
  __syncthreads();
  if (w < 4) {
    double sum = red[0][w][lane];
    for (int x = 1; x < 16; ++x) sum += red[x][w][lane];
    const int row = (lane >> 4) + 4 * w, oc = blockIdx.y * 16 + (lane & 15);
    if (t0 + row < nrows && oc <= d) {
      const int trow = t0 + row;
      int it = rows ? rows[trow] : trow;
      if ((unsigned)it >= (unsigned)nitems) it = 0;
      const size_t o = scatter ? (size_t)it : (size_t)trow;
      P[o * PS + oc] = (float)sum;
    }
  }
}


#define FWD_ARGS (const uint16_t *)h->Ft, rows, (int)nrows, h->cfg.num_items, Deq, (const uint16_t *)h->Et, Pout, h->PS, h->errflag
template <int NT>
void launch_fwd_rows(bprx_handle *h, const int32_t *rows, int64_t nrows, const int32_t *nrows_dev, int scatter, float *Pout,
                     hipStream_t s) {
  const bool f8 = h->cfg.feat_dtype == BPRX_F_FP8;
  const int Deq = f8 ? h->cfg.feat_dim / 2 : h->cfg.feat_dim;
  const float *pscale = h->qs + 1;
  const int64_t tiles = (nrows + 15) / 16;
  const int ncu = h->num_cu > 0 ? h->num_cu : 256;
  int mt = 1;
  if (NT <= 5 && tiles > 8 * (int64_t)ncu) mt = 4;
  else if (NT <= 9 && tiles > 2 * (int64_t)ncu) mt = 2;
  bool split = NT > 1 && tiles * NT <= 2 * (int64_t)ncu;
#define ROWS_LAUNCH(NTW_, MT_, NW_, F8_, GY_)                                                                            \
  do {                                                                                                                   \
    auto kfn = k_proj_fwd_rows<NTW_, MT_, NW_, F8_>;                                                                     \
    const size_t lds = (size_t)NTW_ * 2048 * NW_ / 4;                                                                    \
    if (lds > 48 * 1024) (void)hipFuncSetAttribute((const void *)kfn, hipFuncAttributeMaxDynamicSharedMemorySize, (int)lds); \
    hipLaunchKernelGGL(kfn, dim3((unsigned)((tiles + MT_ - 1) / MT_), (unsigned)(GY_)), dim3(NW_ * 64), lds, s,          \
                       (const uint16_t *)h->Ft, rows, (int)nrows, nrows_dev, h->cfg.num_items, Deq,                      \
                       (const uint16_t *)h->EtF, Pout, h->PS, h->errflag, pscale, scatter);                              \
  } while (0)
  if (split) { if (f8) ROWS_LAUNCH(1, 1, 16, true, NT); else ROWS_LAUNCH(1, 1, 16, false, NT); return; }
  if constexpr (NT <= 5) {
    if (mt == 4) { if (f8) ROWS_LAUNCH(NT, 4, 8, true, 1); else ROWS_LAUNCH(NT, 4, 8, false, 1); return; }
  }
  if constexpr (NT <= 9) {
    if (mt == 2) { if (f8) ROWS_LAUNCH(NT, 2, 8, true, 1); else ROWS_LAUNCH(NT, 2, 8, false, 1); return; }
  }
  if (f8) ROWS_LAUNCH(NT, 1, 8, true, 1); else ROWS_LAUNCH(NT, 1, 8, false, 1);
#undef ROWS_LAUNCH
}

inline bool fwd_nt_loads(const bprx_handle *h) {
  const size_t bytes = (size_t)h->cfg.num_items * h->cfg.feat_dim * (h->cfg.feat_dtype == BPRX_F_FP8 ? 1 : 2);
  return h->cfg.feat_dtype == BPRX_F_BF16 ? true : bytes > ((size_t)256 << 20);
}

template <int NT>
void launch_f8s(bprx_handle *h, const int32_t *rows, int64_t nrows, const int32_t *nrows_dev, int scatter, float *Pout, hipStream_t s,
                int stagger) {
  const float *pscale = h->qs + 1;
  const int64_t T = (nrows + 15) / 16;
  const int ncu = h->num_cu > 0 ? h->num_cu : 256;
  int64_t G = (T + 15) / 16;
  if (G < ncu) G = T < ncu ? T : ncu;
  else G = (G + ncu - 1) / ncu * ncu;
  const size_t lds = (size_t)2 * NT * 2048 + 8 * 4096;
  const bool ntl = fwd_nt_loads(h);
#define F8S_LAUNCH(NTL_)                                                                                                  \
  do {                                                                                                                    \
    auto kfn = k_proj_fwd_f8s<NT, NTL_>;                                                                                  \
    (void)hipFuncSetAttribute((const void *)kfn, hipFuncAttributeMaxDynamicSharedMemorySize, (int)lds);                   \
    hipLaunchKernelGGL(kfn, dim3((unsigned)G), dim3(512), lds, s, (const unsigned char *)h->Ft, (int)nrows, h->cfg.feat_dim,  \
                       (const unsigned char *)h->EtS, Pout, h->PS, pscale, stagger, rows, nrows_dev, scatter, h->cfg.num_items, \
                       h->errflag);                                                                                        \
  } while (0)
  if (ntl) F8S_LAUNCH(true); else F8S_LAUNCH(false);
#undef F8S_LAUNCH
}

template <int NT>
void launch_v10(bprx_handle *h, int64_t nrows, float *Pout, hipStream_t s, int n0) {
  constexpr int NWMAX = 8, NWMIN = 5;
  const bool f8 = h->cfg.feat_dtype == BPRX_F_FP8;
  const int Deq = f8 ? h->cfg.feat_dim / 2 : h->cfg.feat_dim;
  const float *pscale = h->qs + 1;
  const int64_t T = (nrows + 15) / 16;
  const int ncu = h->num_cu > 0 ? h->num_cu : 256;
  int64_t G = (T + 2 * NWMAX - 1) / (2 * NWMAX);
  if (G < ncu) G = T < ncu ? T : ncu;
  else G = (G + ncu - 1) / ncu * ncu;
  const int tpw_max = (int)((T + G - 1) / G);
  const int per_wave = tpw_max > NWMAX ? 2 : 1;
  int nw = (tpw_max + per_wave - 1) / per_wave;
  if (nw < NWMIN) nw = NWMIN;
  const size_t lds = (size_t)2 * NT * 16 * 288 + (size_t)nw * 2 * 16 * 288;
  const bool ntl = fwd_nt_loads(h);
#define V10_LAUNCH(F8_, NTL_)                                                                                             \
  do {                                                                                                                    \
    auto kfn = k_proj_fwd_bf16_v10<NT, F8_, NTL_>;                                                                        \
    (void)hipFuncSetAttribute((const void *)kfn, hipFuncAttributeMaxDynamicSharedMemorySize, (int)lds);                   \
    hipLaunchKernelGGL(kfn, dim3((unsigned)G), dim3(nw * 64), lds, s, (const uint16_t *)h->Ft, (int)nrows, Deq,            \
                       (const uint16_t *)h->Et, Pout, h->PS, pscale, 0, per_wave, n0);                                     \
  } while (0)
  if (f8) { if (ntl) V10_LAUNCH(true, true); else V10_LAUNCH(true, false); }
  else { if (ntl) V10_LAUNCH(false, true); else V10_LAUNCH(false, false); }
#undef V10_LAUNCH
}

template <int NT>
int launch_fwd_nt(bprx_handle *h, const int32_t *rows, int64_t nrows, float *Pout, hipStream_t s) {
  constexpr int MTD = NT <= 9 ? 2 : 1;
  const bool f8 = h->cfg.feat_dtype == BPRX_F_FP8;
  const int Deq = f8 ? h->cfg.feat_dim / 2 : h->cfg.feat_dim;
  const float *pscale = h->qs + 1;
  const bool plain = h->fwd_variant == 0 || Deq % 256 != 0 || rows;
  if (!plain) {
    if constexpr (NT >= 10) {
      if (f8 && h->EtS && h->cfg.feat_dim % 256 == 0) {
        launch_f8s<NT>(h, nullptr, nrows, nullptr, 0, Pout, s, 1);
        return 0;
      }
      for (int c0 = 0; c0 < NT; c0 += 9) launch_v10<9>(h, nrows, Pout, s, (c0 + 9 <= NT ? c0 : NT - 9) * 16);
      return 0;
    } else {
      launch_v10<NT>(h, nrows, Pout, s, 0);
      return 0;
    }
  }
  dim3 grid((unsigned)((nrows + 4 * MTD * 16 - 1) / (4 * MTD * 16)));
  if (f8) hipLaunchKernelGGL((k_proj_fwd_bf16<NT, MTD, true>), grid, dim3(256), 0, s, FWD_ARGS, 0, pscale);
  else hipLaunchKernelGGL((k_proj_fwd_bf16<NT, MTD, false>), grid, dim3(256), 0, s, FWD_ARGS, 0, pscale);
  return 0;
}

template <int NT, int BTV, int NW, int PD, bool F8, bool ROWS, int DB, int NS = 1>
void launch_bwd3(dim3 grid, hipStream_t s, const uint16_t *Ft, int nrows, int D, const uint16_t *Wb, int PS, float *part, int rps,
                 int desc, int xmap, const int32_t *rows, const int32_t *nrows_dev, const float *Wf) {
  constexpr size_t lds = (size_t)DB * (BTV * (NW * 32 * 2 + 32) + BTV * WsStride3<NT>::bytes);
  auto kfn = k_proj_bwd_bf16_v3<NT, BTV, NW, PD, F8, ROWS, DB, NS>;
  if (lds > 48 * 1024) {
    static bool attr_set = false;
    if (!attr_set) { (void)hipFuncSetAttribute((const void *)kfn, hipFuncAttributeMaxDynamicSharedMemorySize, (int)lds); attr_set = true; }
  }
  hipLaunchKernelGGL(kfn, grid, dim3(NW * 64), lds, s, Ft, nrows, D, Wb, PS, part, rps, desc, xmap, rows, nrows_dev, Wf);
}

template <int NT>
int launch_bwd_rows(bprx_handle *h, int64_t bound, hipStream_t s) {
  const int D = h->cfg.feat_dim;
  const bool f8 = h->cfg.feat_dtype == BPRX_F_FP8;
  const bool w8 = D % 256 == 0 || f8;
  dim3 g3(D / (w8 ? 256 : 128), h->SK_step);
#define BWDR_LAUNCH(NW_, F8_)                                                                                            \
  launch_bwd3<NT, 32, NW_, 2, F8_, true, 1>(g3, s, (const uint16_t *)h->Ft, (int)bound, D, (const uint16_t *)h->Wb, h->PS,     \
                                            h->part, 0, 0, 1, (const int32_t *)h->ilist, (const int32_t *)h->list_cur,        \
                                            (const float *)h->W)
  if (f8) BWDR_LAUNCH(8, true);
  else if (w8) BWDR_LAUNCH(8, false);
  else BWDR_LAUNCH(4, false);
#undef BWDR_LAUNCH
  return 0;
}

template <int NT>
int launch_bwd_nt(bprx_handle *h, hipStream_t s) {
  const int D = h->cfg.feat_dim, I = h->cfg.num_items;
  int rps3 = (I + h->SK - 1) / h->SK;
  rps3 = (rps3 + 31) / 32 * 32;
  const size_t n4 = (size_t)I * h->PS / 4;
  if (!h->item_mode)
    hipLaunchKernelGGL(k_cast_W, dim3(1024), dim3(256), 0, s, h->W, (uint16_t *)h->Wb, n4);
  const bool f8 = h->cfg.feat_dtype == BPRX_F_FP8;
  const bool w8 = D % 256 == 0 || f8;
  dim3 g3(D / (w8 ? 256 : 128), h->SK);
#define BWD3_ARGS (const uint16_t *)h->Ft, I, D, (const uint16_t *)h->Wb, h->PS, h->part, rps3, 0, 1, (const int32_t *)nullptr, \
                  (const int32_t *)nullptr, (const float *)nullptr
  if constexpr (NT > 9) {
    if (f8) { launch_bwd3<NT, 32, 8, 2, true, false, 2, 2>(g3, s, BWD3_ARGS); return 0; }
    if (w8) { launch_bwd3<NT, 32, 8, 2, false, false, 2, 2>(g3, s, BWD3_ARGS); return 0; }
  }
  if constexpr (NT <= 9) {
    if (f8) { launch_bwd3<NT, 32, 8, 2, true, false, 2>(g3, s, BWD3_ARGS); return 0; }
    if (w8) { launch_bwd3<NT, 32, 8, 3, false, false, 1>(g3, s, BWD3_ARGS); return 0; }
  }
  launch_bwd3<NT, 32, 4, 2, false, false, 1>(g3, s, BWD3_ARGS);
#undef BWD3_ARGS
  return 0;
}

#define NT_SWITCH(NT, CALL)            \
  switch (NT) {                        \
    case 1: CALL(1); break;            \
    case 2: CALL(2); break;            \
    case 3: CALL(3); break;            \
    case 4: CALL(4); break;            \
    case 5: CALL(5); break;            \
    case 6: CALL(6); break;            \
    case 7: CALL(7); break;            \
    case 8: CALL(8); break;            \
    case 9: CALL(9); break;            \
    case 10: CALL(10); break;          \
    case 11: CALL(11); break;          \
    case 12: CALL(12); break;          \
    case 13: CALL(13); break;          \
    case 14: CALL(14); break;          \
    case 15: CALL(15); break;          \
    case 16: CALL(16); break;          \
    default: CALL(17); break;          \
  }

}

int bprx_launch_tile_F(bprx_handle *h) {
  if (h->cfg.model != BPRX_MODEL_VBPR || h->cfg.feat_dtype == BPRX_F_FP32) return BPRX_OK;
  const int I = h->cfg.num_items, Deq = h->cfg.feat_dtype == BPRX_F_FP8 ? h->cfg.feat_dim / 2 : h->cfg.feat_dim;
  dim3 grid((unsigned)(Deq / 128), (unsigned)((I + 31) / 32));
  hipLaunchKernelGGL(k_tile_F, grid, dim3(256), 0, 0, (const uint16_t *)h->t.F, (uint16_t *)h->Ft, I, Deq);
  BPRX_LAUNCH_CHECK(h, "k_tile_F");
  BPRX_HIP(h, hipStreamSynchronize(0));
  return BPRX_OK;
}

int bprx_launch_cast_Et(bprx_handle *h, hipStream_t s) {
  if (h->cfg.feat_dtype == BPRX_F_FP32) return BPRX_OK;
  if (h->et_valid) return BPRX_OK;
  h->et_valid = true;
  const int D = h->cfg.feat_dim;
  BprxProfScope ps(h, BPRX_PHASE_CAST_ET, s);
  dim3 grid((D + 63) / 64, h->PS / 16);
  if (h->cfg.feat_dtype == BPRX_F_FP8) {
    const int slot = h->qs_slot;
    h->qs_slot ^= 1;
    if (!h->absmax_valid) {
      BPRX_HIP(h, hipMemsetAsync((uint32_t *)h->qs + 2 + slot, 0, sizeof(uint32_t), s));
      hipLaunchKernelGGL(k_absmax, dim3(64), dim3(256), 0, s, h->t.E, (size_t)D * h->cfg.embed_d, h->t.Bp, (size_t)D,
                         (uint32_t *)h->qs + 2 + slot);
    }
    h->absmax_valid = false;
    hipLaunchKernelGGL(k_cast_Et8, dim3((unsigned)((D + 15) / 16)), dim3(256), 0, s, h->t.E, h->t.Bp, (uint8_t *)h->Et,
                       (uint8_t *)h->EtF, (uint8_t *)h->EtS, D, h->cfg.embed_d, h->PS, h->qs, h->cfg.feat_scale, slot);
    BPRX_LAUNCH_CHECK(h, "k_cast_Et8");
    return BPRX_OK;
  }
  hipLaunchKernelGGL(k_cast_Et, grid, dim3(256), 0, s, h->t.E, h->t.Bp, (uint16_t *)h->Et, (uint16_t *)h->EtF, D,
                     h->cfg.embed_d, h->PS);
  BPRX_LAUNCH_CHECK(h, "k_cast_Et");
  return BPRX_OK;
}

int bprx_launch_proj_fwd(bprx_handle *h, const int32_t *rows, int64_t nrows, const int32_t *nrows_dev, int scatter, float *Pout,
                         hipStream_t s) {
  if (nrows <= 0) return BPRX_OK;
  BprxProfScope ps(h, BPRX_PHASE_PROJ_FWD, s);
  if (h->cfg.feat_dtype != BPRX_F_FP32) {
    const int NT = h->PS / 16;
    if (rows && NT >= 10 && h->cfg.feat_dtype == BPRX_F_FP8 && h->EtS && h->cfg.feat_dim % 256 == 0 && nrows >= 4096) {
      switch (NT) {
        case 10: launch_f8s<10>(h, rows, nrows, nrows_dev, scatter, Pout, s, 0); break;
        case 11: launch_f8s<11>(h, rows, nrows, nrows_dev, scatter, Pout, s, 0); break;
        case 12: launch_f8s<12>(h, rows, nrows, nrows_dev, scatter, Pout, s, 0); break;
        case 13: launch_f8s<13>(h, rows, nrows, nrows_dev, scatter, Pout, s, 0); break;
        case 14: launch_f8s<14>(h, rows, nrows, nrows_dev, scatter, Pout, s, 0); break;
        case 15: launch_f8s<15>(h, rows, nrows, nrows_dev, scatter, Pout, s, 0); break;
        case 16: launch_f8s<16>(h, rows, nrows, nrows_dev, scatter, Pout, s, 0); break;
        default: launch_f8s<17>(h, rows, nrows, nrows_dev, scatter, Pout, s, 0); break;
      }
      BPRX_LAUNCH_CHECK(h, "k_proj_fwd_f8s<rows>");
      return BPRX_OK;
    }
    if (rows) {
#define CALL(N) launch_fwd_rows<N>(h, rows, nrows, nrows_dev, scatter, Pout, s)
      NT_SWITCH(NT, CALL)
#undef CALL
      BPRX_LAUNCH_CHECK(h, "k_proj_fwd_rows");
      return BPRX_OK;
    }
#define CALL(N) launch_fwd_nt<N>(h, rows, nrows, Pout, s)
    NT_SWITCH(NT, CALL)
#undef CALL
    BPRX_LAUNCH_CHECK(h, "k_proj_fwd_bf16");
  } else {
    if (h->cfg.feat_dim % 16 == 0) {
      dim3 grid((unsigned)((nrows + 15) / 16), (unsigned)((h->cfg.embed_d + 1 + 15) / 16));
      hipLaunchKernelGGL(k_proj_fwd_f32_mfma, grid, dim3(1024), 0, s, (const float *)h->t.F, rows, (int)nrows, nrows_dev, scatter,
                         h->cfg.num_items, h->cfg.feat_dim, h->t.E, h->t.Bp, h->cfg.embed_d, Pout, h->PS, h->errflag);
    } else {
      dim3 grid((unsigned)((nrows + 3) / 4));
      hipLaunchKernelGGL(k_proj_fwd_f32, grid, dim3(256), 0, s, (const float *)h->t.F, rows, (int)nrows, nrows_dev, scatter,
                         h->cfg.num_items, h->cfg.feat_dim, h->t.E, h->t.Bp, h->cfg.embed_d, Pout, h->PS, h->errflag);
    }
    BPRX_LAUNCH_CHECK(h, "k_proj_fwd_f32");
  }
  return BPRX_OK;
}

int bprx_launch_proj_bwd(bprx_handle *h, int64_t B, hipStream_t s) {
  const int D = h->cfg.feat_dim, d = h->cfg.embed_d, I = h->cfg.num_items;
  const int64_t bound = 2 * B < (int64_t)I ? 2 * B : (int64_t)I;
  h->SK_step = h->SK;
  if (h->cfg.feat_dtype != BPRX_F_FP32) {
    const int NT = h->PS / 16;
    if (h->list_mode) {
      int sk = (int)((bound + 127) / 128);
      h->SK_step = sk < 1 ? 1 : (sk > h->SK ? h->SK : sk);
      {
        BprxProfScope ps(h, BPRX_PHASE_PROJ_BWD, s);
#define CALL(N) launch_bwd_rows<N>(h, bound, s)
        NT_SWITCH(NT, CALL)
#undef CALL
      }
      BPRX_LAUNCH_CHECK(h, "k_proj_bwd_bf16_v3<rows>");
    } else {
      BprxProfScope ps(h, BPRX_PHASE_PROJ_BWD, s);
#define CALL(N) launch_bwd_nt<N>(h, s)
      NT_SWITCH(NT, CALL)
#undef CALL
      BPRX_LAUNCH_CHECK(h, "k_proj_bwd_bf16");
    }
    if (h->fused_reduce) return BPRX_OK;
    const size_t n = (size_t)D * h->PS;
    BprxProfScope ps(h, BPRX_PHASE_REDUCE, s);
    hipLaunchKernelGGL(k_reduce_parts, dim3((unsigned)((n + 255) / 256)), dim3(256), 0, s, h->part, h->SK_step, D, d, h->PS, h->dEp,
                       h->cfg.feat_dtype == BPRX_F_FP8 ? 1.0f / h->cfg.feat_scale : 1.0f);
    BPRX_LAUNCH_CHECK(h, "k_reduce_parts");
  } else {
    {
      BprxProfScope ps(h, BPRX_PHASE_PROJ_BWD, s);
      if (h->list_mode && D % F32_KV == 0)
        hipLaunchKernelGGL(k_proj_bwd_f32_tile, dim3(D / F32_KV, (unsigned)((d + 1 + 31) / 32)), dim3(F32_NRS * 32), 0, s, (const float *)h->t.F,
                           (int)bound, D, h->W, d, h->PS, h->dEp, (const int32_t *)h->ilist, (const int32_t *)h->list_cur);
      else
      hipLaunchKernelGGL(k_proj_bwd_f32, dim3(D), dim3(256), 0, s, (const float *)h->t.F, h->list_mode ? (int)bound : I, D, h->W, d,
                         h->PS, h->dEp, h->list_mode ? (const int32_t *)h->ilist : (const int32_t *)nullptr,
                         h->list_mode ? (const int32_t *)h->list_cur : (const int32_t *)nullptr);
    }
    BPRX_LAUNCH_CHECK(h, "k_proj_bwd_f32");
  }
  return BPRX_OK;
}
```

include/bprx.h:

```cpp
#ifndef BPRX_H_
#define BPRX_H_

#include <stdint.h>

#ifdef __cplusplus
extern "C" {
#endif

#define BPRX_ABI_VERSION 6

#if defined(__GNUC__)
#define BPRX_API __attribute__((visibility("default")))
#else
#define BPRX_API
#endif

enum { BPRX_MODEL_BPRMF = 0, BPRX_MODEL_VBPR = 1 };
enum { BPRX_OPT_SGD = 0, BPRX_OPT_ADAM_TF23 = 1 };
enum { BPRX_F_FP32 = 0, BPRX_F_BF16 = 1, BPRX_F_FP8 = 2 };

enum {
  BPRX_OK = 0,
  BPRX_E_INVALID = -1,
  BPRX_E_STATE = -2,
  BPRX_E_HIP = -3,
  BPRX_E_RANGE = -4,
  BPRX_E_NOMEM = -5
};

typedef struct bprx_handle bprx_handle;
typedef struct bprx_sampler bprx_sampler;

typedef struct {
  int32_t abi_version;
  int32_t model;
  int32_t num_users;
  int32_t num_items;
  int32_t embed_k;
  int32_t embed_d;
  int32_t feat_dim;
  int32_t feat_dtype;
  int32_t optimizer;
  int32_t device;
  int64_t max_batch;
  float lr;
  float reg;
  float beta1, beta2, epsilon;
  int32_t flags;
  float feat_scale;
} bprx_config;

enum { BPRX_FLAG_EXPORT_USER_GRAD = 1, BPRX_FLAG_EXPORT_ITEM_GRAD = 2, BPRX_FLAG_DENSE_ALLREDUCE = 4,
       BPRX_FLAG_ADAM_SWEEP = 8, BPRX_FLAG_ADAM_LAZY = 16 };

typedef struct {
  float *Gu;
  float *Gi;
  float *Bi;
  float *Tu;
  const void *F;
  float *E;
  float *Bp;
  float *m_Gu, *v_Gu, *m_Gi, *v_Gi, *m_Bi, *v_Bi, *m_Tu, *v_Tu, *m_E, *v_E, *m_Bp, *v_Bp;
} bprx_tables;

BPRX_API int bprx_abi_version(void);

BPRX_API int bprx_create(const bprx_config *cfg, bprx_handle **out);
BPRX_API int bprx_destroy(bprx_handle *h);
BPRX_API const char *bprx_last_error(const bprx_handle *h);

BPRX_API int bprx_bind_tables(bprx_handle *h, const bprx_tables *t);
BPRX_API int bprx_tables_dirty(bprx_handle *h, void *stream);
BPRX_API int bprx_set_hyper(bprx_handle *h, float lr, float reg);
BPRX_API int bprx_set_adam_step(bprx_handle *h, int64_t iterations, void *stream);
BPRX_API int bprx_sync_adam(bprx_handle *h, void *stream);
BPRX_API int64_t bprx_get_adam_step(const bprx_handle *h);
BPRX_API int bprx_adam_is_lazy(const bprx_handle *h);

typedef struct {
  int32_t feat_dim_a, feat_dim_b;
  int32_t embed_a, embed_b;
  float neg_bias_reg;
  float *Ea, *Eb, *A, *Ap;
  float *m_Ea, *v_Ea, *m_Eb, *v_Eb, *m_A, *v_A, *m_Ap, *v_Ap;
} bprx_factored;
BPRX_API int bprx_bind_factored(bprx_handle *h, const bprx_tables *t, const bprx_factored *f);
BPRX_API int bprx_explain_pairs(bprx_handle *h, const int32_t *user, const int32_t *item, int64_t n, float *out, void *stream);

enum {
  BPRX_ACF_C_WU = 0, BPRX_ACF_C_WI = 1, BPRX_ACF_C_B0 = 2, BPRX_ACF_C_W1 = 3, BPRX_ACF_C_B1 = 4,
  BPRX_ACF_I_WU = 5, BPRX_ACF_I_WV = 6, BPRX_ACF_I_WP = 7, BPRX_ACF_I_WX = 8, BPRX_ACF_I_B0 = 9,
  BPRX_ACF_I_W1 = 10, BPRX_ACF_I_B1 = 11, BPRX_ACF_NW = 12
};
typedef struct {
  int32_t feat_m, feat_c;
  int32_t width_c, width_i;
  int32_t feat_dtype;
  const void *F;
  const int64_t *train_ptr;
  const int32_t *train_items;
  const int64_t *eval_ptr;
  const int32_t *eval_items;
  float *Pi, *m_Pi, *v_Pi;
  float *w[BPRX_ACF_NW];
  float *m_w[BPRX_ACF_NW], *v_w[BPRX_ACF_NW];
} bprx_acf;
BPRX_API int bprx_bind_acf(bprx_handle *h, const bprx_tables *t, const bprx_acf *a);
BPRX_API int bprx_acf_profiles(bprx_handle *h, const int32_t *users, int64_t n, const int64_t *hist_ptr,
                               const int32_t *hist_items, float *out, void *stream);
BPRX_API int bprx_acf_explain(bprx_handle *h, const int32_t *user, const int32_t *item, int64_t n, const int64_t *hist_ptr,
                              const int32_t *hist_items, int32_t top, float *score, float *base, int32_t *pos,
                              int32_t *hist_item, float *alpha, float *contrib, int32_t *peak, float *beta_peak, float *beta,
                              void *stream);
enum { BPRX_ACF_GRAD_DETACHED = 0, BPRX_ACF_GRAD_FULL = 1 };
BPRX_API int bprx_acf_set_gradient(bprx_handle *h, int mode);
BPRX_API int bprx_acf_get_gradient(bprx_handle *h);

enum {
  BPRX_AF_COL_W1 = 0, BPRX_AF_COL_B1 = 1, BPRX_AF_COL_W2 = 2,
  BPRX_AF_EDG_CW = 3, BPRX_AF_EDG_CB = 4, BPRX_AF_EDG_W2 = 5,
  BPRX_AF_CLS_W1 = 6, BPRX_AF_CLS_B1 = 7, BPRX_AF_CLS_W2 = 8,
  BPRX_AF_ATT_W1 = 9, BPRX_AF_ATT_B1 = 10, BPRX_AF_ATT_W2 = 11, BPRX_AF_ATT_B2 = 12,
  BPRX_AF_NW = 13
};
#define BPRX_AF_IMG 224
#define BPRX_AF_HID 256
#define BPRX_AF_CH 64
typedef struct {
  int32_t dim_color, dim_class;
  int32_t width;
  float dropout;
  uint64_t seed;
  const uint8_t *edges;
  const float *color;
  const float *cls;
  float *w[BPRX_AF_NW];
  float *m_w[BPRX_AF_NW], *v_w[BPRX_AF_NW];
} bprx_attentive;
BPRX_API int bprx_bind_attentive(bprx_handle *h, const bprx_tables *t, const bprx_attentive *a);
BPRX_API int bprx_af_encode(bprx_handle *h, const int32_t *items, int64_t n, float *out, void *stream);
BPRX_API int bprx_af_attention_pairs(bprx_handle *h, const int32_t *user, const int32_t *item, int64_t n, float *x, float *alpha,
                                     void *stream);
BPRX_API int bprx_af_explain(bprx_handle *h, const int32_t *user, const int32_t *item, int64_t n, int32_t grid, float *x,
                             float *alpha, float *parts, float *map, int32_t *peak_cell, float *peak_val, void *stream);
BPRX_API int bprx_af_score_block(bprx_handle *h, int32_t u0, int32_t u1, float *scores, float *alpha, void *stream);
BPRX_API int bprx_af_dropout_mask(bprx_handle *h, int64_t step, int64_t n_rows, uint8_t *out, void *stream);
BPRX_API int64_t bprx_af_get_step(const bprx_handle *h);
BPRX_API int bprx_af_set_step(bprx_handle *h, int64_t step);

BPRX_API int bprx_score_pairs(bprx_handle *h, const int32_t *user, const int32_t *item, int64_t B, float *x, void *stream);

BPRX_API int bprx_step(bprx_handle *h, const int32_t *user, const int32_t *pos, const int32_t *neg, int64_t B,
              float *loss_out, void *stream);

BPRX_API int bprx_step_begin(bprx_handle *h, const int32_t *user, const int32_t *pos, const int32_t *neg, int64_t B,
                    void *stream);
BPRX_API int bprx_dense_grad(bprx_handle *h, float **ptr, int64_t *count);
BPRX_API int bprx_step_end(bprx_handle *h, float *loss_out, void *stream);
BPRX_API int bprx_step_begin_sparse(bprx_handle *h, const int32_t *user, const int32_t *pos, const int32_t *neg, int64_t B,
                           void *stream);
BPRX_API int bprx_step_begin_dense(bprx_handle *h, void *stream);
BPRX_API int bprx_step_project(bprx_handle *h, void *stream);
BPRX_API int bprx_user_grad(bprx_handle *h, float **dGu, float **dTu);
BPRX_API int bprx_clear_user_grad(bprx_handle *h, int64_t n_rows, int32_t marks_only, void *stream);
BPRX_API int64_t bprx_user_msg_floats(const bprx_handle *h, int64_t cap);
BPRX_API int bprx_pack_user_msg(bprx_handle *h, const int32_t *user, int64_t B, int64_t cap, float *msg, void *stream);
BPRX_API int bprx_apply_user_msgs(bprx_handle *h, const float *msgs, int32_t nranks, int64_t cap, float scale, void *stream);
BPRX_API int bprx_sum_dense_parts(bprx_handle *h, const float *parts, int32_t nranks, void *stream);
BPRX_API int bprx_adam_rows(float *p, float *m, float *v, float *g, int64_t n, float lr_t, float beta1, float beta2, float eps,
                            void *stream);
BPRX_API int bprx_step_lr(const bprx_handle *h, float *lr_t);
BPRX_API int bprx_item_grad(bprx_handle *h, float **dGi, float **dBi);
BPRX_API int bprx_clear_item_grad(bprx_handle *h, int64_t n_rows, int32_t marks_only, void *stream);
BPRX_API int bprx_scatter_add(float *table, int32_t num_rows, int32_t num_cols, const int32_t *idx, const float *rows,
                              int64_t n, float scale, void *stream);

BPRX_API int bprx_route_reset(int32_t *send_idx, int64_t nslots, int32_t *cursor, int32_t nranks, void *stream);
BPRX_API int bprx_route_plan(const int32_t *ids, int64_t n, const int32_t *ids_b, int64_t n_b, int32_t rows_per_rank, int32_t nranks,
                             int32_t cap, int32_t my_rank, int32_t *slot, int32_t *send_idx, int32_t *cursor, int32_t *overflow,
                             int32_t *own_cnt, void *stream);
BPRX_API int bprx_route_gather(const float *t0, int32_t w0, const float *t1, int32_t w1, int32_t num_rows, const int32_t *idx,
                               int64_t n, float *out, int32_t *cnt, void *stream);
BPRX_API int bprx_route_unpack(const float *got, const int32_t *slot, int64_t n, float *dst0, int32_t w0, float *dst1, int32_t w1,
                               const float *own0, const float *own1, int32_t own_rows, void *stream);
BPRX_API int bprx_route_gather_checked(const float *t0, int32_t w0, const float *t1, int32_t w1, int32_t num_rows,
                                       const int32_t *idx, int64_t n, float *out, int32_t *cnt, int32_t *err, void *stream);
BPRX_API int bprx_route_unpack_checked(const float *got, const int32_t *slot, int64_t n, float *dst0, int32_t w0, float *dst1,
                                       int32_t w1, const float *own0, const float *own1, int32_t own_rows, int32_t *err, void *stream);
BPRX_API int bprx_route_pack(float *src0, int32_t w0, float *src1, int32_t w1, const int32_t *slot, int64_t n, float *send,
                             float *own0, float *own1, int32_t own_rows, float scale, int32_t *own_cnt, int32_t *send_idx,
                             int64_t nslots, int32_t *cursor, int32_t nranks, void *stream);
BPRX_API int bprx_route_scatter_add(float *t0, int32_t w0, float *t1, int32_t w1, int32_t num_rows, const int32_t *idx,
                                    const float *rows, int64_t n, float scale, int32_t *cnt, void *stream);

BPRX_API int bprx_score_block(bprx_handle *h, int32_t u0, int32_t u1, float *out, void *stream);

enum {
  BPRX_PHASE_CAST_ET = 0, BPRX_PHASE_PROJ_FWD = 1, BPRX_PHASE_TRIPLET = 2, BPRX_PHASE_PROJ_BWD = 3,
  BPRX_PHASE_REDUCE = 4, BPRX_PHASE_APPLY = 5, BPRX_PHASE_DENSE = 6, BPRX_PHASE_LOSS = 7, BPRX_PHASE_ITEM_SEG = 8,
  BPRX_PHASE_SEG_ALLOC = 9, BPRX_PHASE_ROW_COUNT = 10, BPRX_PHASE_ADAM_CATCHUP = 11, BPRX_PHASE_COUNT = 12
};
BPRX_API int bprx_profile_enable(bprx_handle *h, int on);
BPRX_API int bprx_profile_read(bprx_handle *h, double *ms, int64_t *launches);

BPRX_API int bprx_eval_users(bprx_handle *h, int32_t u0, int32_t u1, const float *scores, const int64_t *train_ptr,
                             const int32_t *train_items, const int64_t *eval_ptr, const int32_t *eval_items, int32_t K,
                             double *out, void *stream);

BPRX_API int bprx_eval_pos(bprx_handle *h, int32_t u0, int32_t u1, const float *scores, int32_t item_lo, int32_t items_total,
                           const int64_t *eval_ptr, const int32_t *eval_items, float *sp, void *stream);
BPRX_API int bprx_eval_counts(bprx_handle *h, int32_t u0, int32_t u1, const float *scores, int32_t item_lo, int32_t items_total,
                              const int64_t *train_ptr, const int32_t *train_items, const int64_t *eval_ptr,
                              const int32_t *eval_items, const float *sp, int32_t *counts, void *stream);
BPRX_API int bprx_eval_finish(bprx_handle *h, int32_t u0, int32_t u1, int32_t items_total, const int64_t *eval_ptr,
                              const float *sp, const int32_t *counts, int32_t K, double *out, void *stream);

BPRX_API int bprx_topk(bprx_handle *h, int32_t u0, int32_t u1, float *scores, const int64_t *train_ptr,
                       const int32_t *train_items, int32_t K, int32_t *idx, float *val, int32_t *flag, void *stream);

BPRX_API int64_t bprx_probe_stream_read(const void *buf, int64_t bytes, void *sink, void *stream);
BPRX_API int64_t bprx_probe_stream_read_nt(const void *buf, int64_t bytes, void *sink, void *stream);
BPRX_API int64_t bprx_probe_row_gather(void *table, int64_t num_rows, int32_t row_floats, const int32_t *idx, int64_t n,
                                       int32_t mode, void *sink, void *stream);

BPRX_API int bprx_sync_check(bprx_handle *h, void *stream);

BPRX_API int bprx_sampler_create(const int64_t *indptr, const int32_t *items, int32_t num_users, int32_t num_items,
                        bprx_sampler **out);
BPRX_API int bprx_sampler_destroy(bprx_sampler *s);
BPRX_API int64_t bprx_sampler_count(const bprx_sampler *s, int32_t batch_size, int32_t epochs);
BPRX_API int64_t bprx_sampler_ref_stream(bprx_sampler *s, int32_t batch_size, int32_t epochs, uint32_t py_seed,
                                uint32_t np_seed, int32_t *user, int32_t *pos, int32_t *neg, int64_t cap);

BPRX_API int bprx_sample_philox(const int64_t *indptr, const int32_t *items_sorted, const int32_t *pos_user,
                                int64_t num_pos, int32_t num_items, uint64_t seed, uint64_t first, int64_t B,
                                int32_t *user, int32_t *pos, int32_t *neg, void *stream);

BPRX_API int bprx_epoch_prepare(uint64_t seed, uint32_t epoch, int32_t num_users, const int64_t *indptr, int32_t *perm,
                                int64_t *lens, void *stream);
BPRX_API int bprx_epoch_slots(const int64_t *epoch_ptr, int32_t num_users, int32_t *pos_slot, int64_t num_pos, void *stream);
BPRX_API int bprx_sample_epoch(const int64_t *indptr, const int32_t *items_sorted, const int32_t *perm,
                               const int64_t *epoch_ptr, const int32_t *pos_slot, int32_t num_users, int32_t num_items, uint64_t seed,
                               uint32_t epoch, int64_t first, int64_t B, int32_t *user, int32_t *pos, int32_t *neg,
                               void *stream);

BPRX_API int bprx_sample_philox_h(bprx_handle *h, const int64_t *indptr, const int32_t *items_sorted, const int32_t *pos_user,
                                  int64_t num_pos, int32_t num_items, uint64_t seed, uint64_t first, int64_t B, int32_t *user,
                                  int32_t *pos, int32_t *neg, int64_t batch_offset, int64_t batch_size, void *stream);
BPRX_API int bprx_sample_epoch_h(bprx_handle *h, const int64_t *indptr, const int32_t *items_sorted, const int32_t *perm,
                                 const int64_t *epoch_ptr, const int32_t *pos_slot, int32_t num_users, int32_t num_items,
                                 uint64_t seed, uint32_t epoch, int64_t first, int64_t B, int32_t *user, int32_t *pos, int32_t *neg,
                                 int64_t batch_offset, int64_t batch_size, void *stream);
BPRX_API int bprx_index_pass_kind(const bprx_handle *h);

#ifdef __cplusplus
}
#endif
#endif
```

Baseline: 312.3 million.

## Skip feature loads for untouched items in projection passes via occupancy mask

In item-segment mode, the index pass now runs before the projection forward, and its per-item occupancy counts are passed to both the forward and backward visual projection kernels. These kernels use buffer loads with an out-of-bounds offset, so feature rows for items not in the batch read as zero without touching memory. The goal is to cut feature-table bandwidth when the batch touches only a fraction of the items. In exchange, the index pass is reordered ahead of the forward projection and the backward kernel builds an extra LDS bitmask. The masked path is on by default only for bf16 with a small projection width.

```diff
diff --git a/fashionvisualexpl_recommend_amd/_ffi.py b/fashionvisualexpl_recommend_amd/_ffi.py
--- a/fashionvisualexpl_recommend_amd/_ffi.py
+++ b/fashionvisualexpl_recommend_amd/_ffi.py
@@ -153,6 +153,7 @@
         "bprx_epoch_slots": (C.c_int, [vp, i32, vp, i64, vp]),
         "bprx_sample_epoch": (C.c_int, [vp, vp, vp, vp, vp, i32, i32, C.c_uint64, u32, i64, i64, vp, vp, vp, vp]),
         "bprx_index_pass_kind": (C.c_int, [vp]),
+        "bprx_proj_mask_kind": (C.c_int, [vp]),
         "bprx_adam_rows": (C.c_int, [vp, vp, vp, vp, i64, C.c_float, C.c_float, C.c_float, C.c_float, vp]),
         "bprx_step_lr": (C.c_int, [vp, vp]),
         "bprx_sample_philox_h": (C.c_int, [vp, vp, vp, vp, i64, i32, C.c_uint64, C.c_uint64, i64, vp, vp, vp, i64, i64, vp]),
@@ -179,7 +180,7 @@
            "bprx_scatter_add", "bprx_route_reset", "bprx_route_plan", "bprx_route_gather", "bprx_route_unpack", "bprx_route_gather_checked",
            "bprx_route_unpack_checked", "bprx_route_pack",
            "bprx_route_scatter_add", "bprx_score_block", "bprx_eval_users", "bprx_eval_pos", "bprx_eval_counts", "bprx_eval_finish", "bprx_topk", "bprx_sync_check", "bprx_probe_stream_read", "bprx_probe_stream_read_nt", "bprx_probe_row_gather", "bprx_profile_enable",
-           "bprx_profile_read", "bprx_sample_philox", "bprx_epoch_prepare", "bprx_epoch_slots", "bprx_sample_epoch", "bprx_sample_philox_h", "bprx_sample_epoch_h", "bprx_index_pass_kind", "bprx_adam_rows", "bprx_step_lr", "bprx_user_msg_floats", "bprx_pack_user_msg",
+           "bprx_profile_read", "bprx_sample_philox", "bprx_epoch_prepare", "bprx_epoch_slots", "bprx_sample_epoch", "bprx_sample_philox_h", "bprx_sample_epoch_h", "bprx_index_pass_kind", "bprx_proj_mask_kind", "bprx_adam_rows", "bprx_step_lr", "bprx_user_msg_floats", "bprx_pack_user_msg",
            "bprx_apply_user_msgs", "bprx_sampler_create",
            "bprx_sampler_destroy", "bprx_sampler_count", "bprx_sampler_ref_stream"]
 
diff --git a/fashionvisualexpl_recommend_amd/csrc/bprx_api.hip b/fashionvisualexpl_recommend_amd/csrc/bprx_api.hip
--- a/fashionvisualexpl_recommend_amd/csrc/bprx_api.hip
+++ b/fashionvisualexpl_recommend_amd/csrc/bprx_api.hip
@@ -120,6 +120,7 @@
     if (h->SK > 64) h->SK = 64;
     if (h->SK < 1) h->SK = 1;
     h->fwd_variant = env_int("BPRX_FWD_VARIANT", 4);
+    h->proj_mask = std::min(std::max(env_int("BPRX_PROJ_MASK", 1), 0), 2);
     A(dalloc_zero(&h->dTu, U * d));
     A(dalloc_zero(&h->P, I * PS));
     A(dalloc_zero(&h->W, I * PS));
@@ -376,7 +377,7 @@
   const bool vb = h->cfg.model == BPRX_MODEL_VBPR;
   if (B == 0) {
     if (!(h->cfg.flags & (BPRX_FLAG_EXPORT_USER_GRAD | BPRX_FLAG_EXPORT_ITEM_GRAD))) BPRX_FAIL(h, BPRX_E_INVALID, "step: empty batch");
-    h->list_mode = 0; h->item_mode = 0;
+    h->list_mode = 0; h->item_mode = 0; h->step_masked = false; h->mask_kind = 0;
     if (h->cfg.optimizer == BPRX_OPT_ADAM_TF23) {
       h->adam_t += 1;
       const float t = (float)h->adam_t;
@@ -394,6 +395,7 @@
   if (!user || !pos || !neg) BPRX_FAIL(h, BPRX_E_INVALID, "step: null index pointer");
   h->list_mode = vb && !h->proj_fresh && (h->list_policy == 2 || (h->list_policy == 1 && 2 * B < (int64_t)h->cfg.num_items));
   h->item_mode = !h->list_mode && (h->seg_policy == 2 || (h->seg_policy == 1 && 2 * B >= (int64_t)h->cfg.num_items));
+  h->step_masked = false;
   h->list_reset_cnt = !(h->fast_rows && !(h->cfg.flags & BPRX_FLAG_EXPORT_ITEM_GRAD));
   h->idx8_use = h->idx8_ready(pos, neg, B);
   h->idx8_n = 0;
@@ -423,12 +425,18 @@
     if (!h->p_valid &&
         (rc = bprx_launch_proj_fwd(h, h->ilist, h->list_bound, h->list_cur, 1, h->P, s))) return rc;
   } else if (vb && !h->proj_fresh) {
+    h->step_masked = h->item_mode && !h->p_valid &&
+                     (h->proj_mask == 2 ? h->cfg.feat_dtype != BPRX_F_FP32
+                                        : (h->proj_mask == 1 && h->cfg.feat_dtype == BPRX_F_BF16 && h->PS / 16 <= 9));
+    if (h->step_masked && (rc = bprx_launch_index_pass(h, user, pos, neg, B, s))) return rc;
     if ((rc = bprx_launch_cast_Et(h, s))) return rc;
-    if (!h->p_valid && (rc = bprx_launch_proj_fwd(h, nullptr, h->cfg.num_items, nullptr, 0, h->P, s))) return rc;
-  }
+    if (!h->p_valid && (rc = bprx_launch_proj_fwd(h, nullptr, h->cfg.num_items, nullptr, 0, h->P, s,
+                                                  h->step_masked ? h->seg_cnt : nullptr))) return rc;
+  }
+  h->mask_kind = h->step_masked && h->fwd_masked ? 2 : 0;
   h->proj_fresh = false;
   if (catchup_aside) BPRX_HIP(h, hipStreamWaitEvent(s, h->ev_join, 0));
-  if (!h->list_mode && (rc = bprx_launch_index_pass(h, user, pos, neg, B, s))) return rc;
+  if (!h->list_mode && !h->step_masked && (rc = bprx_launch_index_pass(h, user, pos, neg, B, s))) return rc;
   if ((rc = bprx_launch_triplet_grad(h, user, pos, neg, B, s))) return rc;
   h->pending_B = B;
   h->pending_stage = 1;
@@ -451,7 +459,8 @@
   const float lr_t = h->pend_lr;
   int rc;
   if ((rc = bprx_launch_item_seg(h, pos, neg, B, lr_t, s))) return rc;
-  if (vb && (rc = bprx_launch_proj_bwd(h, B, s))) return rc;
+  if (vb && (rc = bprx_launch_proj_bwd(h, B, s, h->step_masked ? h->seg_cnt : nullptr))) return rc;
+  if (vb) h->mask_kind = h->mask_kind == 2 ? (h->bwd_masked ? 1 : 2) : (h->bwd_masked ? 3 : 0);
   if ((rc = bprx_launch_apply(h, user, pos, neg, B, lr_t, s))) return rc;
   h->pending_stage = 2;
   return BPRX_OK;
@@ -589,6 +598,7 @@
 }
 
 extern "C" int bprx_index_pass_kind(const bprx_handle *h) { return h ? h->idx_kind : 0; }
+extern "C" int bprx_proj_mask_kind(const bprx_handle *h) { return h ? h->mask_kind : 0; }
 
 extern "C" int bprx_sync_check(bprx_handle *h, void *stream) {
   if (!h) return BPRX_E_INVALID;
diff --git a/fashionvisualexpl_recommend_amd/csrc/bprx_internal.h b/fashionvisualexpl_recommend_amd/csrc/bprx_internal.h
--- a/fashionvisualexpl_recommend_amd/csrc/bprx_internal.h
+++ b/fashionvisualexpl_recommend_amd/csrc/bprx_internal.h
@@ -72,6 +72,10 @@
   int64_t idx8_B, idx8_n;
   bool idx8_use;
   int idx_kind;
+  int proj_mask;
+  bool step_masked;
+  bool fwd_masked, bwd_masked;
+  int mask_kind;
   bool idx8_ready(const int32_t *pos, const int32_t *neg, int64_t B) const {
     return item_mode && own8 && B > 0 && idx8_n == B && idx8_B == B && idx8_pos == pos && idx8_neg == neg && B % 16 == 0;
   }
@@ -166,8 +170,8 @@
 int bprx_launch_tile_F(bprx_handle *h);
 int bprx_launch_cast_Et(bprx_handle *h, hipStream_t s);
 int bprx_launch_proj_fwd(bprx_handle *h, const int32_t *rows, int64_t nrows, const int32_t *nrows_dev, int scatter, float *Pout,
-                         hipStream_t s);
-int bprx_launch_proj_bwd(bprx_handle *h, int64_t B, hipStream_t s);
+                         hipStream_t s, const int32_t *occ = nullptr);
+int bprx_launch_proj_bwd(bprx_handle *h, int64_t B, hipStream_t s, const int32_t *occ = nullptr);
 int bprx_launch_fact_compose(bprx_handle *h, hipStream_t s);
 int bprx_launch_fact_update(bprx_handle *h, float lr_t, hipStream_t s);
 int bprx_launch_explain(bprx_handle *h, const int32_t *u, const int32_t *i, int64_t n, float *out, hipStream_t s);
diff --git a/fashionvisualexpl_recommend_amd/csrc/bprx_proj.hip b/fashionvisualexpl_recommend_amd/csrc/bprx_proj.hip
--- a/fashionvisualexpl_recommend_amd/csrc/bprx_proj.hip
+++ b/fashionvisualexpl_recommend_amd/csrc/bprx_proj.hip
@@ -29,6 +29,18 @@
 __device__ __forceinline__ i32x4_t ld_stream16(const void *p) {
   if constexpr (NT) return __builtin_nontemporal_load(reinterpret_cast<const i32x4_t *>(p));
   else return *reinterpret_cast<const i32x4_t *>(p);
+}
+constexpr uint32_t BUF_OOB = 0x80000000u;
+__device__ __forceinline__ __amdgpu_buffer_rsrc_t ft_rsrc(const void *base, uint32_t bytes) {
+  const uintptr_t b = (uintptr_t)base;
+  const uintptr_t u = (uintptr_t)(uint32_t)__builtin_amdgcn_readfirstlane((int)(uint32_t)b) |
+                      ((uintptr_t)(uint32_t)__builtin_amdgcn_readfirstlane((int)(uint32_t)(b >> 32)) << 32);
+  return __builtin_amdgcn_make_buffer_rsrc(reinterpret_cast<void *>(u), 0, __builtin_amdgcn_readfirstlane((int)bytes),
+                                           0x00020000);
+}
+template <bool NT>
+__device__ __forceinline__ i32x4_t ld_buf16(__amdgpu_buffer_rsrc_t rs, uint32_t voff, uint32_t soff) {
+  return __builtin_amdgcn_raw_buffer_load_b128(rs, (int)voff, __builtin_amdgcn_readfirstlane((int)soff), NT ? 2 : 0);
 }
 template <bool F8>
 __device__ __forceinline__ f32x4 mfma_frag(i32x4_t a, i32x4_t b, f32x4 c) {
@@ -327,13 +339,14 @@
   o1 = __builtin_bit_cast(uint32_t, __builtin_amdgcn_cvt_scalef32_pk_bf16_fp8(w, 1.0f, true));
 }
 
-template <int NT, int BTV, int NW, int PD, bool F8, bool ROWS = false, int DB = 1, int NS = 1>
+template <int NT, int BTV, int NW, int PD, bool F8, bool ROWS = false, int DB = 1, int NS = 1, bool MASK = false>
 __global__ __launch_bounds__(NW * 64) void k_proj_bwd_bf16_v3(const uint16_t *__restrict__ F, int nrows, int D,
                                                           const uint16_t *__restrict__ Wb, int PS, float *__restrict__ part,
                                                           int rows_per_split, int descend, int xcd_map,
                                                           const int32_t *__restrict__ rows = nullptr,
                                                           const int32_t *__restrict__ nrows_dev = nullptr,
-                                                          const float *__restrict__ Wf = nullptr) {
+                                                          const float *__restrict__ Wf = nullptr,
+                                                          const int32_t *__restrict__ occ = nullptr) {
   constexpr int NTH = NW * 64, MC = NW * 32;
   constexpr int ESZ = F8 ? 1 : 2;
   constexpr int FCH = MC * ESZ / 16;
@@ -376,6 +389,10 @@
     for (int nt = 0; nt < NTW; ++nt) acc[mt][nt] = f32x4{0.f, 0.f, 0.f, 0.f};
   uint4 freg[PD][FPT], wreg[PD][WPT];
   uint4 wreg2[ROWS ? PD : 1][WPT];
+  static_assert(!(MASK && ROWS), "the row-list form has no untouched rows");
+  uint32_t *const tmask = reinterpret_cast<uint32_t *>(lds_bwd3 + DB * IMG);
+  const __amdgpu_buffer_rsrc_t frs = ft_rsrc(F + (size_t)(tbeg >> 5) * (Deq >> 7) * 4096,
+                                             MASK ? (uint32_t)(ntiles * (BTV / 32)) * (uint32_t)(Deq >> 7) * 8192u : 0u);
 #define BWD3_ISSUE(ST, TILE)                                                                                             \
   {                                                                                                                      \
     int tile_ = (TILE);                                                                                                  \
@@ -392,8 +409,16 @@
                                                        (size_t)(pp & 15) * 8);                                           \
       } else {                                                                                                           \
         const size_t bidx = (size_t)((t0 >> 5) + blk / CBK) * (Deq >> 7) + (m0q >> 7) + blk % CBK;                       \
-        { const i32x4_t v_ = ld_stream16<!F8>(F + bidx * 4096 + (size_t)(pp & 511) * 8);                                 \
-          freg[ST][x] = make_uint4((unsigned)v_.x, (unsigned)v_.y, (unsigned)v_.z, (unsigned)v_.w); }                      \
+        i32x4_t v_;                                                                                                      \
+        if constexpr (MASK) {                                                                                            \
+          const uint32_t br_ = (uint32_t)(((t0 - tbeg) >> 5) + blk / CBK);               \
+          const uint32_t on_ = (tmask[br_] >> ((pp & 511) >> 4)) & 1u;                                                   \
+          v_ = ld_buf16<!F8>(frs, on_ ? (uint32_t)((m0q >> 7) + blk % CBK) * 8192u + (uint32_t)(pp & 511) * 16u : BUF_OOB, \
+                             br_ * (uint32_t)(Deq >> 7) * 8192u);                                                        \
+        } else {                                                                                                         \
+          v_ = ld_stream16<!F8>(F + bidx * 4096 + (size_t)(pp & 511) * 8);                                               \
+        }                                                                                                                \
+        freg[ST][x] = make_uint4((unsigned)v_.x, (unsigned)v_.y, (unsigned)v_.z, (unsigned)v_.w);                        \
       }                                                                                                                  \
     }                                                                                                                    \
     _Pragma("unroll") for (int x = 0; x < WPT; ++x) {                                                                    \
@@ -457,6 +482,16 @@
     for (int e = threadIdx.x; e < MC * PS; e += NTH) slab0[e] = 0.f;
     return;
   }
+  if constexpr (MASK) {
+    {
+      for (int r0 = w * 64; r0 < ntiles * BTV; r0 += NTH) {
+        const int t = tbeg + r0 + lane;
+        const unsigned long long b = __ballot(t < tend && occ[t] != 0);
+        if (lane == 0) { tmask[r0 >> 5] = (uint32_t)b; tmask[(r0 >> 5) + 1] = (uint32_t)(b >> 32); }
+      }
+      __syncthreads();
+    }
+  }
 #pragma unroll
   for (int st = 0; st < PD; ++st) BWD3_ISSUE(st, st)
   for (int tile0 = 0; tile0 < ntiles; tile0 += PD) {
@@ -507,8 +542,9 @@
 }
 
 
-template <int NT, int MT, bool F8, bool NTL>
-__device__ __forceinline__ void v10_body(const uint16_t *const (&asrc)[2], const uint16_t *__restrict__ Et, unsigned char *lds,
+template <int NT, int MT, bool F8, bool NTL, bool MASK>
+__device__ __forceinline__ void v10_body(const uint16_t *const (&asrc)[2], const uint32_t (&voff)[2][4],
+                                         const uint16_t *__restrict__ Et, unsigned char *lds,
                                          unsigned char *myA, f32x4 (&acc)[2][NT], int D, int cshift, int lane, int et_chunk) {
   constexpr int BSB = (KC + 16) * 2;
   constexpr int BBUF = NT * 16 * BSB;
@@ -520,12 +556,17 @@
   i32x4_t aX[MT][4], aY[MT][4];
   constexpr int NBR = (NPIECE + 319) / 320;
   i32x4_t bst[NBR];
+  __amdgpu_buffer_rsrc_t ars[MT];
+#pragma unroll
+  for (int mt = 0; mt < MT; ++mt) ars[mt] = ft_rsrc(asrc[mt], MASK ? (uint32_t)nch * 8192u : 0u);
 #define V10_ISSUE(c_, AR)                                                                                             \
   {                                                                                                                   \
     int ce_ = (c_) + cshift;                                                                                          \
     if (ce_ >= nch) ce_ -= nch;                                                                                       \
-    _Pragma("unroll") for (int mt = 0; mt < MT; ++mt) _Pragma("unroll") for (int x = 0; x < 4; ++x)                   \
-        AR[mt][x] = ld_stream16<NTL>(asrc[mt] + ((size_t)ce_ << 12) + x * 512 + lane * 8);                          \
+    _Pragma("unroll") for (int mt = 0; mt < MT; ++mt) _Pragma("unroll") for (int x = 0; x < 4; ++x) {                 \
+      if constexpr (MASK) AR[mt][x] = ld_buf16<NTL>(ars[mt], voff[mt][x], (uint32_t)ce_ << 13);   \
+      else AR[mt][x] = ld_stream16<NTL>(asrc[mt] + ((size_t)ce_ << 12) + x * 512 + lane * 8);                        \
+    }                                                                                                                 \
     const uint16_t *bc_ = Et + (size_t)ce_ * et_chunk;                                                                \
     _Pragma("unroll") for (int x = 0; x < NBR; ++x) {                                                                 \
       int pc = tid + x * bdim;                                                                                        \
@@ -580,11 +621,11 @@
 #undef V10_COMPUTE
 }
 
-template <int NT, bool F8, bool NTL>
+template <int NT, bool F8, bool NTL, bool MASK>
 __global__ __launch_bounds__(512) void k_proj_fwd_bf16_v10(const uint16_t *__restrict__ F, int nrows, int D,
                                                            const uint16_t *__restrict__ Et, float *__restrict__ P, int PS,
                                                            const float *__restrict__ pscale, int stagger, int tiles_per_wave,
-                                                           int n0) {
+                                                           int n0, const int32_t *__restrict__ occ) {
   extern __shared__ __attribute__((aligned(16))) unsigned char lds_v10[];
   constexpr int BSB = (KC + 16) * 2;
   const int lane = threadIdx.x & 63, w = __builtin_amdgcn_readfirstlane(threadIdx.x >> 6);
@@ -594,11 +635,17 @@
   const int first = t0 + w * tiles_per_wave;
   const int nlive = (first < t1 ? 1 : 0) + ((tiles_per_wave == 2 && first + 1 < t1) ? 1 : 0);
   const uint16_t *asrc[2];
+  uint32_t voff[2][4];
 #pragma unroll
   for (int mt = 0; mt < 2; ++mt) {
     int tile = first + mt;
     if (tile >= t1) tile = t1 > t0 ? t1 - 1 : 0;
     asrc[mt] = F + ft_row(tile * 16, D);
+#pragma unroll
+    for (int x = 0; x < 4; ++x) {
+      const int t = tile * 16 + x * 4 + q;
+      voff[mt][x] = (MASK && t < nrows && occ[t] != 0) ? (uint32_t)(x * 1024 + lane * 16) : BUF_OOB;
+    }
   }
   f32x4 acc[2][NT];
 #pragma unroll
@@ -608,8 +655,8 @@
   const int nch = D / KC;
   const int cshift = (stagger & 1) ? (int)(blockIdx.x % (unsigned)nch) : 0;
   unsigned char *myA = lds_v10 + 2 * NT * 16 * BSB + w * (2 * 16 * BSB);
-  if (nlive == 2) v10_body<NT, 2, F8, NTL>(asrc, Et + (size_t)n0 * 128, lds_v10, myA, acc, D, cshift, lane, PS * 128);
-  else v10_body<NT, 1, F8, NTL>(asrc, Et + (size_t)n0 * 128, lds_v10, myA, acc, D, cshift, lane, PS * 128);
+  if (nlive == 2) v10_body<NT, 2, F8, NTL, MASK>(asrc, voff, Et + (size_t)n0 * 128, lds_v10, myA, acc, D, cshift, lane, PS * 128);
+  else v10_body<NT, 1, F8, NTL, MASK>(asrc, voff, Et + (size_t)n0 * 128, lds_v10, myA, acc, D, cshift, lane, PS * 128);
   const float ps = F8 ? *pscale : 1.0f;
 #pragma unroll
   for (int mt = 0; mt < 2; ++mt) {
@@ -1003,7 +1050,7 @@
 }
 
 template <int NT>
-void launch_v10(bprx_handle *h, int64_t nrows, float *Pout, hipStream_t s, int n0) {
+void launch_v10(bprx_handle *h, int64_t nrows, float *Pout, hipStream_t s, int n0, const int32_t *occ) {
   constexpr int NWMAX = 8, NWMIN = 5;
   const bool f8 = h->cfg.feat_dtype == BPRX_F_FP8;
   const int Deq = f8 ? h->cfg.feat_dim / 2 : h->cfg.feat_dim;
@@ -1019,35 +1066,43 @@
   if (nw < NWMIN) nw = NWMIN;
   const size_t lds = (size_t)2 * NT * 16 * 288 + (size_t)nw * 2 * 16 * 288;
   const bool ntl = fwd_nt_loads(h);
-#define V10_LAUNCH(F8_, NTL_)                                                                                             \
+#define V10_LAUNCH(F8_, NTL_, MASK_)                                                                                      \
   do {                                                                                                                    \
-    auto kfn = k_proj_fwd_bf16_v10<NT, F8_, NTL_>;                                                                        \
+    auto kfn = k_proj_fwd_bf16_v10<NT, F8_, NTL_, MASK_>;                                                                 \
     (void)hipFuncSetAttribute((const void *)kfn, hipFuncAttributeMaxDynamicSharedMemorySize, (int)lds);                   \
     hipLaunchKernelGGL(kfn, dim3((unsigned)G), dim3(nw * 64), lds, s, (const uint16_t *)h->Ft, (int)nrows, Deq,            \
-                       (const uint16_t *)h->Et, Pout, h->PS, pscale, 0, per_wave, n0);                                     \
+                       (const uint16_t *)h->Et, Pout, h->PS, pscale, 0, per_wave, n0, occ);                                \
   } while (0)
-  if (f8) { if (ntl) V10_LAUNCH(true, true); else V10_LAUNCH(true, false); }
-  else { if (ntl) V10_LAUNCH(false, true); else V10_LAUNCH(false, false); }
+  if (occ) {
+    if (f8) { if (ntl) V10_LAUNCH(true, true, true); else V10_LAUNCH(true, false, true); }
+    else { if (ntl) V10_LAUNCH(false, true, true); else V10_LAUNCH(false, false, true); }
+  } else {
+    if (f8) { if (ntl) V10_LAUNCH(true, true, false); else V10_LAUNCH(true, false, false); }
+    else { if (ntl) V10_LAUNCH(false, true, false); else V10_LAUNCH(false, false, false); }
+  }
 #undef V10_LAUNCH
 }
 
 template <int NT>
-int launch_fwd_nt(bprx_handle *h, const int32_t *rows, int64_t nrows, float *Pout, hipStream_t s) {
+int launch_fwd_nt(bprx_handle *h, const int32_t *rows, int64_t nrows, float *Pout, hipStream_t s, const int32_t *occ) {
   constexpr int MTD = NT <= 9 ? 2 : 1;
   const bool f8 = h->cfg.feat_dtype == BPRX_F_FP8;
   const int Deq = f8 ? h->cfg.feat_dim / 2 : h->cfg.feat_dim;
   const float *pscale = h->qs + 1;
   const bool plain = h->fwd_variant == 0 || Deq % 256 != 0 || rows;
+  h->fwd_masked = false;
   if (!plain) {
     if constexpr (NT >= 10) {
       if (f8 && h->EtS && h->cfg.feat_dim % 256 == 0) {
         launch_f8s<NT>(h, nullptr, nrows, nullptr, 0, Pout, s, 1);
         return 0;
       }
-      for (int c0 = 0; c0 < NT; c0 += 9) launch_v10<9>(h, nrows, Pout, s, (c0 + 9 <= NT ? c0 : NT - 9) * 16);
+      for (int c0 = 0; c0 < NT; c0 += 9) launch_v10<9>(h, nrows, Pout, s, (c0 + 9 <= NT ? c0 : NT - 9) * 16, occ);
+      h->fwd_masked = occ != nullptr;
       return 0;
     } else {
-      launch_v10<NT>(h, nrows, Pout, s, 0);
+      launch_v10<NT>(h, nrows, Pout, s, 0, occ);
+      h->fwd_masked = occ != nullptr;
       return 0;
     }
   }
@@ -1057,16 +1112,16 @@
   return 0;
 }
 
-template <int NT, int BTV, int NW, int PD, bool F8, bool ROWS, int DB, int NS = 1>
+template <int NT, int BTV, int NW, int PD, bool F8, bool ROWS, int DB, int NS = 1, bool MASK = false>
 void launch_bwd3(dim3 grid, hipStream_t s, const uint16_t *Ft, int nrows, int D, const uint16_t *Wb, int PS, float *part, int rps,
-                 int desc, int xmap, const int32_t *rows, const int32_t *nrows_dev, const float *Wf) {
-  constexpr size_t lds = (size_t)DB * (BTV * (NW * 32 * 2 + 32) + BTV * WsStride3<NT>::bytes);
-  auto kfn = k_proj_bwd_bf16_v3<NT, BTV, NW, PD, F8, ROWS, DB, NS>;
+                 int desc, int xmap, const int32_t *rows, const int32_t *nrows_dev, const float *Wf, const int32_t *occ = nullptr) {
+  const size_t lds = (size_t)DB * (BTV * (NW * 32 * 2 + 32) + BTV * WsStride3<NT>::bytes) + (MASK ? ((size_t)rps / 32 + 2) * 4 : 0);
+  auto kfn = k_proj_bwd_bf16_v3<NT, BTV, NW, PD, F8, ROWS, DB, NS, MASK>;
   if (lds > 48 * 1024) {
-    static bool attr_set = false;
-    if (!attr_set) { (void)hipFuncSetAttribute((const void *)kfn, hipFuncAttributeMaxDynamicSharedMemorySize, (int)lds); attr_set = true; }
-  }
-  hipLaunchKernelGGL(kfn, grid, dim3(NW * 64), lds, s, Ft, nrows, D, Wb, PS, part, rps, desc, xmap, rows, nrows_dev, Wf);
+    static size_t attr_lds = 0;
+    if (lds > attr_lds) { (void)hipFuncSetAttribute((const void *)kfn, hipFuncAttributeMaxDynamicSharedMemorySize, (int)lds); attr_lds = lds; }
+  }
+  hipLaunchKernelGGL(kfn, grid, dim3(NW * 64), lds, s, Ft, nrows, D, Wb, PS, part, rps, desc, xmap, rows, nrows_dev, Wf, occ);
 }
 
 template <int NT>
@@ -1087,7 +1142,7 @@
 }
 
 template <int NT>
-int launch_bwd_nt(bprx_handle *h, hipStream_t s) {
+int launch_bwd_nt(bprx_handle *h, hipStream_t s, const int32_t *occ) {
   const int D = h->cfg.feat_dim, I = h->cfg.num_items;
   int rps3 = (I + h->SK - 1) / h->SK;
   rps3 = (rps3 + 31) / 32 * 32;
@@ -1097,19 +1152,27 @@
   const bool f8 = h->cfg.feat_dtype == BPRX_F_FP8;
   const bool w8 = D % 256 == 0 || f8;
   dim3 g3(D / (w8 ? 256 : 128), h->SK);
+  if (rps3 / 32 > 4096 || (size_t)rps3 * D * (h->cfg.feat_dtype == BPRX_F_FP8 ? 1 : 2) >= ((size_t)1 << 31)) occ = nullptr;
+  h->bwd_masked = occ != nullptr;
 #define BWD3_ARGS (const uint16_t *)h->Ft, I, D, (const uint16_t *)h->Wb, h->PS, h->part, rps3, 0, 1, (const int32_t *)nullptr, \
-                  (const int32_t *)nullptr, (const float *)nullptr
+                  (const int32_t *)nullptr, (const float *)nullptr, occ
+#define BWD3_GO(...)                                                                  \
+  do {                                                                                \
+    if (occ) launch_bwd3<__VA_ARGS__, true>(g3, s, BWD3_ARGS);                        \
+    else launch_bwd3<__VA_ARGS__, false>(g3, s, BWD3_ARGS);                           \
+    return 0;                                                                         \
+  } while (0)
   if constexpr (NT > 9) {
-    if (f8) { launch_bwd3<NT, 32, 8, 2, true, false, 2, 2>(g3, s, BWD3_ARGS); return 0; }
-    if (w8) { launch_bwd3<NT, 32, 8, 2, false, false, 2, 2>(g3, s, BWD3_ARGS); return 0; }
+    if (f8) BWD3_GO(NT, 32, 8, 2, true, false, 2, 2);
+    if (w8) BWD3_GO(NT, 32, 8, 2, false, false, 2, 2);
   }
   if constexpr (NT <= 9) {
-    if (f8) { launch_bwd3<NT, 32, 8, 2, true, false, 2>(g3, s, BWD3_ARGS); return 0; }
-    if (w8) { launch_bwd3<NT, 32, 8, 3, false, false, 1>(g3, s, BWD3_ARGS); return 0; }
-  }
-  launch_bwd3<NT, 32, 4, 2, false, false, 1>(g3, s, BWD3_ARGS);
+    if (f8) BWD3_GO(NT, 32, 8, 2, true, false, 2, 1);
+    if (w8) BWD3_GO(NT, 32, 8, 3, false, false, 1, 1);
+  }
+  BWD3_GO(NT, 32, 4, 2, false, false, 1, 1);
+#undef BWD3_GO
 #undef BWD3_ARGS
-  return 0;
 }
 
 #define NT_SWITCH(NT, CALL)            \
@@ -1173,7 +1236,8 @@
 }
 
 int bprx_launch_proj_fwd(bprx_handle *h, const int32_t *rows, int64_t nrows, const int32_t *nrows_dev, int scatter, float *Pout,
-                         hipStream_t s) {
+                         hipStream_t s, const int32_t *occ) {
+  h->fwd_masked = false;
   if (nrows <= 0) return BPRX_OK;
   BprxProfScope ps(h, BPRX_PHASE_PROJ_FWD, s);
   if (h->cfg.feat_dtype != BPRX_F_FP32) {
@@ -1199,7 +1263,7 @@
       BPRX_LAUNCH_CHECK(h, "k_proj_fwd_rows");
       return BPRX_OK;
     }
-#define CALL(N) launch_fwd_nt<N>(h, rows, nrows, Pout, s)
+#define CALL(N) launch_fwd_nt<N>(h, rows, nrows, Pout, s, occ)
     NT_SWITCH(NT, CALL)
 #undef CALL
     BPRX_LAUNCH_CHECK(h, "k_proj_fwd_bf16");
@@ -1218,7 +1282,8 @@
   return BPRX_OK;
 }
 
-int bprx_launch_proj_bwd(bprx_handle *h, int64_t B, hipStream_t s) {
+int bprx_launch_proj_bwd(bprx_handle *h, int64_t B, hipStream_t s, const int32_t *occ) {
+  h->bwd_masked = false;
   const int D = h->cfg.feat_dim, d = h->cfg.embed_d, I = h->cfg.num_items;
   const int64_t bound = 2 * B < (int64_t)I ? 2 * B : (int64_t)I;
   h->SK_step = h->SK;
@@ -1236,7 +1301,7 @@
       BPRX_LAUNCH_CHECK(h, "k_proj_bwd_bf16_v3<rows>");
     } else {
       BprxProfScope ps(h, BPRX_PHASE_PROJ_BWD, s);
-#define CALL(N) launch_bwd_nt<N>(h, s)
+#define CALL(N) launch_bwd_nt<N>(h, s, occ)
       NT_SWITCH(NT, CALL)
 #undef CALL
       BPRX_LAUNCH_CHECK(h, "k_proj_bwd_bf16");
diff --git a/include/bprx.h b/include/bprx.h
--- a/include/bprx.h
+++ b/include/bprx.h
@@ -253,6 +253,7 @@
                                  uint64_t seed, uint32_t epoch, int64_t first, int64_t B, int32_t *user, int32_t *pos, int32_t *neg,
                                  int64_t batch_offset, int64_t batch_size, void *stream);
 BPRX_API int bprx_index_pass_kind(const bprx_handle *h);
+BPRX_API int bprx_proj_mask_kind(const bprx_handle *h);
 
 #ifdef __cplusplus
 }
```

Result: faster. 315.7 million (median of 6 runs) (+1.1%).
